# xiaoxiaokuye/CODLAD

Measured on NVIDIA B200. Metric: backmapped residues/sec (100-step, 10-ensemble), higher is better.
Workload: dtype f16 (tcgen05, fp32 accumulate)

## Files before the change

codlad_b200/csrc/capi.cu:

```cuda
#include <stdarg.h>
#include <string.h>

#include <map>
#include <string>
#include <vector>

#include "../../include/codlad_b200.h"
#include "decode.h"
#include "model.h"

namespace cb2 {

static thread_local char g_err[1024] = "";

void set_error(const char* fmt, ...) {
    va_list ap;
    va_start(ap, fmt);
    vsnprintf(g_err, sizeof(g_err), fmt, ap);
    va_end(ap);
}

float* plan_P(Plan& p, int which) { return p.P + (size_t)which * p.NB * p.L * 256; }

namespace {

struct TensorTable {
    std::map<std::string, const cb2_tensor*> by_name;
    TensorTable(const cb2_tensor* t, int n) {
        for (int i = 0; i < n; ++i) by_name[t[i].name] = &t[i];
    }
    const float* get(const std::string& name, long long numel) const {
        auto it = by_name.find(name);
        if (it == by_name.end()) { set_error("missing tensor '%s'", name.c_str()); return nullptr; }
        if (it->second->numel != numel) {
            set_error("tensor '%s': numel %lld, expected %lld", name.c_str(), it->second->numel, numel);
            return nullptr;
        }
        return it->second->data;
    }
};

struct Packer {
    std::vector<float> buf;
    size_t reserve(size_t n) {
        size_t off = (buf.size() + 63) & ~(size_t)63;
        buf.resize(off + n, 0.0f);
        return off;
    }
    size_t transposed(const float* W, int out, int in_total, int col0, int ncols, float scale = 1.0f) {
        size_t off = reserve((size_t)ncols * out);
        for (int k = 0; k < ncols; ++k)
            for (int o = 0; o < out; ++o) buf[off + (size_t)k * out + o] = scale * W[(size_t)o * in_total + col0 + k];
        return off;
    }
    size_t copy(const float* v, size_t n) {
        size_t off = reserve(n);
        memcpy(&buf[off], v, n * sizeof(float));
        return off;
    }
};

struct HalfPacker {
    std::vector<__half> buf;
    size_t block(const float* W, int in_total, int col0, float scale = 1.0f) {
        size_t off = buf.size();
        buf.resize(off + 128 * 128);
        for (int o = 0; o < 128; ++o)
            for (int k = 0; k < 128; ++k) buf[off + (size_t)o * 128 + k] = __float2half_rn(scale * W[(size_t)o * in_total + col0 + k]);
        return off;
    }
};

#define GET(var, name, numel)                               \
    const float* var = tt.get(name, (long long)(numel));    \
    if (!var) return 1;

template <typename T>
int dev_alloc(std::vector<void*>& owned, T** ptr, size_t count) {
    void* q = nullptr;
    CB2_CUDA(cudaMalloc(&q, count * sizeof(T) > 0 ? count * sizeof(T) : 16));
    owned.push_back(q);
    *ptr = reinterpret_cast<T*>(q);
    return 0;
}

}
}

using namespace cb2;

struct cb2_denoiser { DenoiserModel m; };
struct cb2_vae { VaeModel v; };
struct cb2_plan {
    Plan p;
    float* ca_full = nullptr;
    int *csr_row = nullptr, *csr_col = nullptr;
    int E = 0;
    signed char* orders = nullptr;
    int* slot_atom = nullptr;
    long long* out_off = nullptr;
    float *edge_w = nullptr, *S40 = nullptr, *phi = nullptr, *ic = nullptr, *zq = nullptr;
    int* vq_idx = nullptr;
    float *xa = nullptr, *xb = nullptr;
    int keep_debug = 0;
    bool frames_ready = false, topo_ready = false;
};

extern "C" {

int cb2_abi_version(void) { return CB2_ABI_VERSION; }
const char* cb2_last_error(void) { return cb2::g_err; }

int cb2_denoiser_create(const cb2_tensor* tensors, int n_tensors, const float* freqs128, int k_neighbors, cb2_denoiser** out) {
    if (!tensors || !freqs128 || !out) { set_error("denoiser_create: null argument"); return 1; }
    TensorTable tt(tensors, n_tensors);
    Packer pk;
    HalfPacker bp;
    const int H = CB2_H;
    std::map<std::string, size_t> off;
    std::map<std::string, size_t> boff;

    off["freqs"] = pk.copy(freqs128, 128);
    GET(te0w, "t_embedder.mlp.0.weight", H * 256) GET(te0b, "t_embedder.mlp.0.bias", H)
    GET(te2w, "t_embedder.mlp.2.weight", H * H) GET(te2b, "t_embedder.mlp.2.bias", H)
    off["te_w0_t"] = pk.transposed(te0w, H, 256, 0, 256); off["te_b0"] = pk.copy(te0b, H);
    off["te_w2_t"] = pk.transposed(te2w, H, H, 0, H); off["te_b2"] = pk.copy(te2b, H);

    {
        size_t wo = pk.reserve((size_t)H * CB2_MOD_TOTAL), bo = pk.reserve(CB2_MOD_TOTAL);
        off["ada_w_t"] = wo; off["ada_b"] = bo;
        int col = 0;
        auto put = [&](const std::string& pre, int width) -> int {
            const float* w = tt.get(pre + ".adaLN_modulation.1.weight", (long long)width * H);
            const float* b = tt.get(pre + ".adaLN_modulation.1.bias", width);
            if (!w || !b) return 1;
            for (int o = 0; o < width; ++o) {
                pk.buf[bo + col + o] = b[o];
                for (int k = 0; k < H; ++k) pk.buf[wo + (size_t)k * CB2_MOD_TOTAL + col + o] = w[(size_t)o * H + k];
            }
            col += width;
            return 0;
        };
        for (int l = 0; l < 3; ++l) if (put("encoder_layers." + std::to_string(l), CB2_MOD_ENC)) return 1;
        for (int l = 0; l < 3; ++l) if (put("decoder_layers." + std::to_string(l), CB2_MOD_DEC)) return 1;
        if (put("W_out", CB2_MOD_FIN)) return 1;
    }
    GET(xinw, "x_in.weight", H * 3) GET(xinb, "x_in.bias", H)
    off["xin_w_t"] = pk.transposed(xinw, H, 3, 0, 3); off["xin_b"] = pk.copy(xinb, H);

    GET(posw, "features.embeddings.linear.weight", 16 * 66) GET(posb, "features.embeddings.linear.bias", 16)
    GET(edgew, "features.edge_embedding.weight", H * 167)
    GET(lnw, "features.norm_edges.weight", H) GET(lnb, "features.norm_edges.bias", H)
    GET(wew, "W_e.weight", H * H) GET(web, "W_e.bias", H)
    {
        size_t o = pk.reserve(65 * H);
        for (int d = 0; d < 65; ++d)
            for (int c = 0; c < H; ++c) {
                double a = 0.0;
                for (int q = 0; q < 16; ++q) a += (double)(posw[q * 66 + d] + posb[q]) * (double)edgew[(size_t)c * 167 + q];
                pk.buf[o + (size_t)d * H + c] = (float)a;
            }
        off["pos_table"] = o;
        size_t w = pk.reserve(152 * H);
        for (int r = 0; r < 151; ++r)
            for (int c = 0; c < H; ++c) pk.buf[w + (size_t)r * H + c] = edgew[(size_t)c * 167 + 16 + r];
        off["wedge_t"] = w;
    }
    off["ln_w"] = pk.copy(lnw, H); off["ln_b"] = pk.copy(lnb, H);
    off["we_t"] = pk.transposed(wew, H, H, 0, H); off["we_b"] = pk.copy(web, H);

    GET(ws, "W_s.weight", 30 * H)
    for (int l = 0; l < 3; ++l) {
        const std::string p = "encoder_layers." + std::to_string(l), k = "e" + std::to_string(l) + ".";
        GET(w1, p + ".W1.weight", H * 3 * H) GET(b1, p + ".W1.bias", H) GET(w2, p + ".W2.weight", H * H) GET(b2, p + ".W2.bias", H)
        GET(w3, p + ".W3.weight", H * H) GET(b3, p + ".W3.bias", H)
        GET(w11, p + ".W11.weight", H * 3 * H) GET(b11, p + ".W11.bias", H) GET(w12, p + ".W12.weight", H * H) GET(b12, p + ".W12.bias", H)
        GET(w13, p + ".W13.weight", H * H) GET(b13, p + ".W13.bias", H)
        GET(win, p + ".dense.W_in.weight", 4 * H * H) GET(bin, p + ".dense.W_in.bias", 4 * H)
        GET(wout, p + ".dense.W_out.weight", H * 4 * H) GET(bout, p + ".dense.W_out.bias", H)
        off[k + "W1a_t"] = pk.transposed(w1, H, 3 * H, 0, H); off[k + "W1b_t"] = pk.transposed(w1, H, 3 * H, H, H);
        off[k + "W1c_t"] = pk.transposed(w1, H, 3 * H, 2 * H, H); off[k + "b1"] = pk.copy(b1, H);
        off[k + "W2_t"] = pk.transposed(w2, H, H, 0, H); off[k + "b2"] = pk.copy(b2, H);
        off[k + "W3_t"] = pk.transposed(w3, H, H, 0, H); off[k + "b3"] = pk.copy(b3, H);
        off[k + "W11a_t"] = pk.transposed(w11, H, 3 * H, 0, H); off[k + "W11b_t"] = pk.transposed(w11, H, 3 * H, H, H);
        off[k + "W11c_t"] = pk.transposed(w11, H, 3 * H, 2 * H, H); off[k + "b11"] = pk.copy(b11, H);
        off[k + "W12_t"] = pk.transposed(w12, H, H, 0, H); off[k + "b12"] = pk.copy(b12, H);
        off[k + "W13_t"] = pk.transposed(w13, H, H, 0, H); off[k + "b13"] = pk.copy(b13, H);
        off[k + "Win_t"] = pk.transposed(win, 4 * H, H, 0, H); off[k + "bin"] = pk.copy(bin, 4 * H);
        off[k + "Wout_t"] = pk.transposed(wout, H, 4 * H, 0, 4 * H); off[k + "bout"] = pk.copy(bout, H);
        boff[k + "W1b"] = bp.block(w1, 3 * H, H); boff[k + "W2"] = bp.block(w2, H, 0, 0.5f);
        boff[k + "W11b"] = bp.block(w11, 3 * H, H); boff[k + "W12"] = bp.block(w12, H, 0, 0.5f); boff[k + "W13"] = bp.block(w13, H, 0, 0.5f);
        boff[k + "W1a"] = bp.block(w1, 3 * H, 0); boff[k + "W1c"] = bp.block(w1, 3 * H, 2 * H);
        boff[k + "W11a"] = bp.block(w11, 3 * H, 0); boff[k + "W11c"] = bp.block(w11, 3 * H, 2 * H);
        boff[k + "W3"] = bp.block(w3, H, 0);
        for (int q = 0; q < 4; ++q) { size_t o = bp.block(win + (size_t)q * H * H, H, 0); if (q == 0) boff[k + "Win"] = o; }
        for (int q = 0; q < 4; ++q) { size_t o = bp.block(wout, 4 * H, q * H, 0.5f); if (q == 0) boff[k + "Wout"] = o; }
    }
    for (int l = 0; l < 3; ++l) {
        const std::string p = "decoder_layers." + std::to_string(l), k = "d" + std::to_string(l) + ".";
        GET(w1, p + ".W1.weight", H * 4 * H) GET(b1, p + ".W1.bias", H) GET(w2, p + ".W2.weight", H * H) GET(b2, p + ".W2.bias", H)
        GET(w3, p + ".W3.weight", H * H) GET(b3, p + ".W3.bias", H)
        GET(win, p + ".dense.W_in.weight", 4 * H * H) GET(bin, p + ".dense.W_in.bias", 4 * H)
        GET(wout, p + ".dense.W_out.weight", H * 4 * H) GET(bout, p + ".dense.W_out.bias", H)
        off[k + "W1a_t"] = pk.transposed(w1, H, 4 * H, 0, H); off[k + "W1b2_t"] = pk.transposed(w1, H, 4 * H, H, H, 2.0f);
        off[k + "W1d_t"] = pk.transposed(w1, H, 4 * H, 3 * H, H); off[k + "b1"] = pk.copy(b1, H);
        {
            size_t o = pk.reserve(30 * H);
            for (int z = 0; z < 30; ++z)
                for (int c = 0; c < H; ++c) {
                    double a = 0.0;
                    for (int q = 0; q < H; ++q) a += (double)ws[z * H + q] * (double)w1[(size_t)c * 4 * H + 2 * H + q];
                    pk.buf[o + (size_t)z * H + c] = (float)(2.0 * a);
                }
            off[k + "TS"] = o;
        }
        off[k + "W2_t"] = pk.transposed(w2, H, H, 0, H); off[k + "b2"] = pk.copy(b2, H);
        off[k + "W3_t"] = pk.transposed(w3, H, H, 0, H); off[k + "b3"] = pk.copy(b3, H);
        off[k + "Win_t"] = pk.transposed(win, 4 * H, H, 0, H); off[k + "bin"] = pk.copy(bin, 4 * H);
        off[k + "Wout_t"] = pk.transposed(wout, H, 4 * H, 0, 4 * H); off[k + "bout"] = pk.copy(bout, H);
        boff[k + "W1b2"] = bp.block(w1, 4 * H, H, 2.0f); boff[k + "W2"] = bp.block(w2, H, 0, 0.5f);
        boff[k + "W1a"] = bp.block(w1, 4 * H, 0); boff[k + "W1d"] = bp.block(w1, 4 * H, 3 * H);
        boff[k + "W3"] = bp.block(w3, H, 0);
        for (int q = 0; q < 4; ++q) { size_t o = bp.block(win + (size_t)q * H * H, H, 0); if (q == 0) boff[k + "Win"] = o; }
        for (int q = 0; q < 4; ++q) { size_t o = bp.block(wout, 4 * H, q * H, 0.5f); if (q == 0) boff[k + "Wout"] = o; }
    }
    GET(finw, "W_out.linear.weight", 6 * H) GET(finb, "W_out.linear.bias", 6)
    off["fin_w_t"] = pk.transposed(finw, 6, H, 0, H); off["fin_b"] = pk.copy(finb, 6);

    cb2_denoiser* d = new cb2_denoiser();
    DenoiserModel& m = d->m;
    m.k_neighbors = k_neighbors;
    CB2_CUDA(cudaMalloc(&m.dev_f32, pk.buf.size() * sizeof(float)));
    CB2_CUDA(cudaMemcpy(m.dev_f32, pk.buf.data(), pk.buf.size() * sizeof(float), cudaMemcpyHostToDevice));
    {
        std::vector<__half> v16;
        std::map<std::string, size_t> voff;
        auto putv = [&](const std::string& key, const float* src) {
            voff[key] = v16.size();
            for (int q = 0; q < H; ++q) v16.push_back(__float2half_rn(src[q]));
        };
        for (int l = 0; l < 3; ++l) {
            const std::string pe = "encoder_layers." + std::to_string(l), pd = "decoder_layers." + std::to_string(l);
            putv("e" + std::to_string(l) + ".b2", tt.get(pe + ".W2.bias", H));
            putv("e" + std::to_string(l) + ".b12", tt.get(pe + ".W12.bias", H));
            putv("e" + std::to_string(l) + ".b13", tt.get(pe + ".W13.bias", H));
            putv("d" + std::to_string(l) + ".b2", tt.get(pd + ".W2.bias", H));
        }
        CB2_CUDA(cudaMalloc(&m.dev_vec16, v16.size() * sizeof(__half)));
        CB2_CUDA(cudaMemcpy(m.dev_vec16, v16.data(), v16.size() * sizeof(__half), cudaMemcpyHostToDevice));
        for (int l = 0; l < 3; ++l) {
            m.enc[l].b2_16 = m.dev_vec16 + voff.at("e" + std::to_string(l) + ".b2");
            m.enc[l].b12_16 = m.dev_vec16 + voff.at("e" + std::to_string(l) + ".b12");
            m.enc[l].b13_16 = m.dev_vec16 + voff.at("e" + std::to_string(l) + ".b13");
            m.dec[l].b2_16 = m.dev_vec16 + voff.at("d" + std::to_string(l) + ".b2");
        }
    }
    CB2_CUDA(cudaMalloc(&m.dev_f16, bp.buf.size() * sizeof(__half)));
    CB2_CUDA(cudaMemcpy(m.dev_f16, bp.buf.data(), bp.buf.size() * sizeof(__half), cudaMemcpyHostToDevice));
    m.n_f16_blocks = (int)(bp.buf.size() / (128 * 128));
    auto F = [&](const std::string& key) { return (const float*)(m.dev_f32 + off.at(key)); };
    auto B = [&](const std::string& key) { return (const __half*)(m.dev_f16 + boff.at(key)); };
    m.freqs = F("freqs"); m.te_w0_t = F("te_w0_t"); m.te_b0 = F("te_b0"); m.te_w2_t = F("te_w2_t"); m.te_b2 = F("te_b2");
    m.ada_w_t = F("ada_w_t"); m.ada_b = F("ada_b"); m.xin_w_t = F("xin_w_t"); m.xin_b = F("xin_b");
    m.pos_table = F("pos_table"); m.wedge_t = F("wedge_t"); m.ln_w = F("ln_w"); m.ln_b = F("ln_b"); m.we_t = F("we_t"); m.we_b = F("we_b");
    for (int l = 0; l < 3; ++l) {
        const std::string k = "e" + std::to_string(l) + ".";
        EncLayerW& e = m.enc[l];
        e.W1a_t = F(k + "W1a_t"); e.W1b_t = F(k + "W1b_t"); e.W1c_t = F(k + "W1c_t"); e.b1 = F(k + "b1");
        e.W2_t = F(k + "W2_t"); e.b2 = F(k + "b2"); e.W3_t = F(k + "W3_t"); e.b3 = F(k + "b3");
        e.W11a_t = F(k + "W11a_t"); e.W11b_t = F(k + "W11b_t"); e.W11c_t = F(k + "W11c_t"); e.b11 = F(k + "b11");
        e.W12_t = F(k + "W12_t"); e.b12 = F(k + "b12"); e.W13_t = F(k + "W13_t"); e.b13 = F(k + "b13");
        e.Win_t = F(k + "Win_t"); e.bin = F(k + "bin"); e.Wout_t = F(k + "Wout_t"); e.bout = F(k + "bout");
        e.W1b_h = B(k + "W1b"); e.W2_h = B(k + "W2"); e.W11b_h = B(k + "W11b"); e.W12_h = B(k + "W12"); e.W13_h = B(k + "W13");
        e.W1a_h = B(k + "W1a"); e.W1c_h = B(k + "W1c"); e.W11a_h = B(k + "W11a"); e.W11c_h = B(k + "W11c");
        e.W3_h = B(k + "W3"); e.Win_h = B(k + "Win"); e.Wout_h = B(k + "Wout");
    }
    for (int l = 0; l < 3; ++l) {
        const std::string k = "d" + std::to_string(l) + ".";
        DecLayerW& e = m.dec[l];
        e.W1a_t = F(k + "W1a_t"); e.W1b2_t = F(k + "W1b2_t"); e.W1d_t = F(k + "W1d_t"); e.b1 = F(k + "b1"); e.TS = F(k + "TS");
        e.W2_t = F(k + "W2_t"); e.b2 = F(k + "b2"); e.W3_t = F(k + "W3_t"); e.b3 = F(k + "b3");
        e.Win_t = F(k + "Win_t"); e.bin = F(k + "bin"); e.Wout_t = F(k + "Wout_t"); e.bout = F(k + "bout");
        e.W1b2_h = B(k + "W1b2"); e.W2_h = B(k + "W2");
        e.W1a_h = B(k + "W1a"); e.W1d_h = B(k + "W1d"); e.W3_h = B(k + "W3"); e.Win_h = B(k + "Win"); e.Wout_h = B(k + "Wout");
    }
    m.fin_w_t = F("fin_w_t"); m.fin_b = F("fin_b");
    *out = d;
    return 0;
}

void cb2_denoiser_destroy(cb2_denoiser* d) {
    if (!d) return;
    cudaFree(d->m.dev_f32);
    cudaFree(d->m.dev_f16);
    cudaFree(d->m.dev_vec16);
    delete d;
}

int cb2_vae_create(const cb2_tensor* tensors, int n_tensors, const float* mean3, const float* std3, int angle_variant, cb2_vae** out) {
    if (!tensors || !mean3 || !std3 || !out) { set_error("vae_create: null argument"); return 1; }
    TensorTable tt(tensors, n_tensors);
    Packer pk;
    std::map<std::string, size_t> off;
    const std::string P = "equivaraintconv.";
    auto itcb = tt.by_name.find("quantize._codebook.embed");
    if (itcb == tt.by_name.end() || itcb->second->numel % 3 != 0) { set_error("missing/invalid quantize._codebook.embed"); return 1; }
    const int M = (int)(itcb->second->numel / 3);
    off["codebook"] = pk.copy(itcb->second->data, (size_t)M * 3);
    off["mean"] = pk.copy(mean3, 3); off["std"] = pk.copy(std3, 3);
    GET(mow, "map_out.weight", 36 * 3) GET(mob, "map_out.bias", 36)
    off["mapw_t"] = pk.transposed(mow, 36, 3, 0, 3); off["mapb"] = pk.copy(mob, 36);
    GET(remb, P + "res_embed.weight", 25 * 4) off["res_embed"] = pk.copy(remb, 100);
    const int D = 40, T = angle_variant ? 50 : 40;
    auto linear = [&](const std::string& key, const std::string& name, int o, int i) -> int {
        const float* w = tt.get(P + name + ".weight", (long long)o * i);
        const float* b = tt.get(P + name + ".bias", o);
        if (!w || !b) return 1;
        off[key + "_t"] = pk.transposed(w, o, i, 0, i);
        off[key + "_b"] = pk.copy(b, o);
        return 0;
    };
    size_t wd = pk.reserve(4 * 15 * D), bd = pk.reserve(4 * D);
    off["Wd_t"] = wd; off["bd"] = bd;
    for (int b = 0; b < 4; ++b) {
        const std::string s = std::to_string(b);
        if (linear("inv0." + s, "message_blocks." + s + ".inv_dense.0", D, D)) return 1;
        if (linear("inv1." + s, "message_blocks." + s + ".inv_dense.1", D, D)) return 1;
        GET(dw, P + "message_blocks." + s + ".dist_embed.block.1.weight", D * 15)
        GET(db, P + "message_blocks." + s + ".dist_embed.block.1.bias", D)
        for (int q = 0; q < 15; ++q)
            for (int c = 0; c < D; ++c) pk.buf[wd + ((size_t)b * 15 + q) * D + c] = dw[c * 15 + q];
        for (int c = 0; c < D; ++c) pk.buf[bd + b * D + c] = db[c];
        if (linear("db1." + s, "dense_blocks." + s + ".1", D, D)) return 1;
        if (linear("db3." + s, "dense_blocks." + s + ".3", D, D)) return 1;
        if (linear("tb1." + s, "sidechain_torsion_blocks." + s + ".1", T, T)) return 1;
        if (linear("tb3." + s, "sidechain_torsion_blocks." + s + ".3", T, T)) return 1;
    }
    GET(bbd, P + "backbone_dist.weight", 75) GET(scd, P + "sidechain_dist.weight", 250)
    off["bb_dist"] = pk.copy(bbd, 75); off["sc_dist"] = pk.copy(scd, 250);
    if (linear("ba1", "backbone_angle.1", 3, D) || linear("ba3", "backbone_angle.3", 3, 3)) return 1;
    if (linear("bt1", "backbone_torsion.1", 3, D + 3) || linear("bt3", "backbone_torsion.3", 3, 3)) return 1;
    if (angle_variant) {
        if (linear("sa1", "sidechain_angle.1", 10, D) || linear("sa3", "sidechain_angle.3", 10, 10)) return 1;
    } else {
        GET(sae, P + "sidechain_angle.weight", 250) off["sa_embed"] = pk.copy(sae, 250);
    }
    if (linear("ft1", "final_torsion.1", 10, T) || linear("ft3", "final_torsion.3", 10, 10)) return 1;

    cb2_vae* h = new cb2_vae();
    VaeModel& v = h->v;
    v.M = M; v.angle_variant = angle_variant;
    CB2_CUDA(cudaMalloc(&v.dev, pk.buf.size() * sizeof(float)));
    CB2_CUDA(cudaMemcpy(v.dev, pk.buf.data(), pk.buf.size() * sizeof(float), cudaMemcpyHostToDevice));
    auto F = [&](const std::string& key) -> const float* {
        auto it = off.find(key);
        return it == off.end() ? nullptr : (const float*)(v.dev + it->second);
    };
    v.codebook = F("codebook"); v.mean = F("mean"); v.stdv = F("std"); v.mapw_t = F("mapw_t"); v.mapb = F("mapb");
    v.res_embed = F("res_embed"); v.Wd_t = F("Wd_t"); v.bd = F("bd");
    for (int b = 0; b < 4; ++b) {
        const std::string s = std::to_string(b);
        v.inv0_t[b] = F("inv0." + s + "_t"); v.inv0_b[b] = F("inv0." + s + "_b");
        v.inv1_t[b] = F("inv1." + s + "_t"); v.inv1_b[b] = F("inv1." + s + "_b");
        v.db1_t[b] = F("db1." + s + "_t"); v.db1_b[b] = F("db1." + s + "_b");
        v.db3_t[b] = F("db3." + s + "_t"); v.db3_b[b] = F("db3." + s + "_b");
        v.tb1_t[b] = F("tb1." + s + "_t"); v.tb1_b[b] = F("tb1." + s + "_b");
        v.tb3_t[b] = F("tb3." + s + "_t"); v.tb3_b[b] = F("tb3." + s + "_b");
    }
    v.bb_dist = F("bb_dist"); v.sc_dist = F("sc_dist"); v.sa_embed = F("sa_embed");
    v.ba1_t = F("ba1_t"); v.ba1_b = F("ba1_b"); v.ba3_t = F("ba3_t"); v.ba3_b = F("ba3_b");
    v.bt1_t = F("bt1_t"); v.bt1_b = F("bt1_b"); v.bt3_t = F("bt3_t"); v.bt3_b = F("bt3_b");
    v.sa1_t = F("sa1_t"); v.sa1_b = F("sa1_b"); v.sa3_t = F("sa3_t"); v.sa3_b = F("sa3_b");
    v.ft1_t = F("ft1_t"); v.ft1_b = F("ft1_b"); v.ft3_t = F("ft3_t"); v.ft3_b = F("ft3_b");
    CB2_CUDA(cudaMalloc(&v.e2, (size_t)M * sizeof(float)));
    if (int e = launch_codebook_norms(v.codebook, M, v.e2, 0)) return e;
    CB2_CUDA(cudaStreamSynchronize(0));
    *out = h;
    return 0;
}

void cb2_vae_destroy(cb2_vae* h) {
    if (!h) return;
    cudaFree(h->v.dev);
    cudaFree(h->v.e2);
    delete h;
}

int cb2_plan_create(const cb2_denoiser* d, int F, int NB, int L, int precision, int keep_debug, cb2_plan** out) {
    if (!out || F <= 0 || NB <= 0 || L <= 0) { set_error("plan_create: bad argument"); return 1; }
    if (precision != PREC_F32 && precision != PREC_F16) { set_error("plan_create: unknown precision %d", precision); return 1; }
    cb2_plan* h = new cb2_plan();
    Plan& p = h->p;
    p.model = d ? &d->m : nullptr; p.F = F; p.NB = NB; p.L = L; p.precision = precision;
    h->keep_debug = keep_debug;
    if (!d) {
        int e = 0;
        e |= dev_alloc(p.allocs, &p.X, (size_t)F * L * 3);
        e |= dev_alloc(p.allocs, &p.lengths, F);
        e |= dev_alloc(p.allocs, &p.cg_z, (size_t)F * L);
        e |= dev_alloc(p.allocs, &p.frame_of, NB);
        if (e) { cb2_plan_destroy(h); return e; }
        *out = h;
        return 0;
    }
    p.K = d->m.k_neighbors < L ? d->m.k_neighbors : L;
    const size_t N = (size_t)NB * L, FE = (size_t)F * L * p.K, NE = N * p.K;
    const size_t esz = precision == PREC_F16 ? 2 : 4;
    int e = 0;
    e |= dev_alloc(p.allocs, &p.X, (size_t)F * L * 3);
    e |= dev_alloc(p.allocs, &p.lengths, F);
    e |= dev_alloc(p.allocs, &p.cg_z, (size_t)F * L);
    e |= dev_alloc(p.allocs, &p.frame_of, NB);
    e |= dev_alloc(p.allocs, &p.nbr_idx, FE);
    e |= dev_alloc(p.allocs, &p.nbr_dist, FE);
    e |= dev_alloc(p.allocs, reinterpret_cast<unsigned char**>(&p.hE0), FE * 128 * esz);
    e |= dev_alloc(p.allocs, reinterpret_cast<unsigned char**>(&p.hE), NE * 128 * esz);
    if (keep_debug) e |= dev_alloc(p.allocs, &p.E_dbg, FE * 128);
    e |= dev_alloc(p.allocs, &p.hV, N * 128);
    e |= dev_alloc(p.allocs, &p.hVenc, N * 128);
    e |= dev_alloc(p.allocs, &p.P, 2 * N * 256);
    if (precision == PREC_F16) {
        e |= dev_alloc(p.allocs, &p.P16[0], N * 256);
        e |= dev_alloc(p.allocs, &p.P16[1], N * 256);
    }
    e |= dev_alloc(p.allocs, &p.S, N * 128);
    e |= dev_alloc(p.allocs, &p.out6, N * 6);
    e |= dev_alloc(p.allocs, &h->xa, N * 3);
    e |= dev_alloc(p.allocs, &h->xb, N * 3);
    p.mod_capacity = NB > 1024 ? NB : 1024;
    e |= dev_alloc(p.allocs, &p.mod, (size_t)p.mod_capacity * CB2_MOD_TOTAL);
    if (precision == PREC_F16) e |= dev_alloc(p.allocs, &p.mod16, (size_t)p.mod_capacity * 768);
    e |= dev_alloc(p.allocs, &p.silu_c, (size_t)p.mod_capacity * 128);
    e |= dev_alloc(p.allocs, &p.tvals, p.mod_capacity);
    e |= dev_alloc(p.allocs, &p.coef, (size_t)p.mod_capacity * 8);
    if (e) { cb2_plan_destroy(h); return e; }
    if (precision == PREC_F16) {
        if (int r = edge_tc_prepare(p)) { cb2_plan_destroy(h); return r; }
        if (int r = node_tc_prepare(p)) { cb2_plan_destroy(h); return r; }
    }
    *out = h;
    return 0;
}

void cb2_plan_destroy(cb2_plan* h) {
    if (!h) return;
    if (h->p.graph) cudaGraphExecDestroy(h->p.graph);
    edge_tc_release(h->p);
    node_tc_release(h->p);
    for (void* q : h->p.allocs) cudaFree(q);
    delete h;
}

int cb2_plan_K(const cb2_plan* h) { return h ? h->p.K : 0; }
long long cb2_plan_launches(const cb2_plan* h) { return h ? h->p.launches : 0; }

int cb2_plan_set_frames(cb2_plan* h, const float* X, const int* lengths, const int* cg_z, const int* frame_of, void* stream) {
    if (!h || !X || !lengths || !cg_z || !frame_of) { set_error("set_frames: null argument"); return 1; }
    Plan& p = h->p;
    cudaStream_t s = (cudaStream_t)stream;
    CB2_CUDA(cudaMemcpyAsync(p.X, X, (size_t)p.F * p.L * 3 * sizeof(float), cudaMemcpyDeviceToDevice, s));
    CB2_CUDA(cudaMemcpyAsync(p.lengths, lengths, p.F * sizeof(int), cudaMemcpyDeviceToDevice, s));
    CB2_CUDA(cudaMemcpyAsync(p.cg_z, cg_z, (size_t)p.F * p.L * sizeof(int), cudaMemcpyDeviceToDevice, s));
    CB2_CUDA(cudaMemcpyAsync(p.frame_of, frame_of, p.NB * sizeof(int), cudaMemcpyDeviceToDevice, s));
    if (p.model == nullptr) { h->frames_ready = true; return 0; }
    {
        std::vector<int> len((size_t)p.F);
        CB2_CUDA(cudaMemcpyAsync(len.data(), p.lengths, (size_t)p.F * sizeof(int), cudaMemcpyDeviceToHost, s));
        CB2_CUDA(cudaStreamSynchronize(s));
        p.all_full = true;
        for (int f = 0; f < p.F; ++f) p.all_full = p.all_full && len[f] >= p.L;
    }
    if (int e = launch_knn(p.X, p.lengths, p.F, p.L, p.K, p.nbr_dist, p.nbr_idx, s)) return e;
    if (int e = launch_edge_features(*p.model, p.X, p.lengths, p.nbr_idx, p.nbr_dist, p.F, p.L, p.K, p.E_dbg, p.hE0, p.precision, s)) return e;
    p.launches += 2;
    h->frames_ready = true;
    return 0;
}

}

namespace {

int edge_dispatch(Plan& p, int mode, int layer, const float* mod_base, int mod_stride, cudaStream_t s) {
    return p.precision == PREC_F16 ? launch_edge_tc(p, mode, layer, mod_base, mod_stride, s)
                                    : launch_edge_f32(p, mode, layer, mod_base, mod_stride, s);
}

int run_forward(Plan& p, const float* x, const float* mod_base, int mod_stride, const float* noise, float* x_next,
                const float* coef_row, cudaStream_t s, int stop_after = -1) {
    int n = 0;
    auto done = [&]() { return stop_after >= 0 && ++n >= stop_after; };
    const bool tc = p.precision == PREC_F16 && p.node_tc != nullptr;
    auto node_update = [&](int phase, const float* xt, const float* nz, float* xn, const float* cf) {
        return tc ? launch_node_update_tc(p, phase, mod_base, mod_stride, xt, nz, xn, cf, s)
                  : launch_node_update(p, phase, mod_base, mod_stride, xt, nz, xn, cf, s);
    };
    if (int e = tc ? launch_node_init_tc(p, x, s) : launch_node_init(p, x, mod_base, mod_stride, s)) return e;
    if (done()) return 0;
    for (int l = 0; l < 3; ++l) {
        if (int e = edge_dispatch(p, EDGE_ENC_NODE, l, mod_base, mod_stride, s)) return e;
        if (done()) return 0;
        if (int e = node_update(l, nullptr, nullptr, nullptr, nullptr)) return e;
        if (done()) return 0;
        if (int e = edge_dispatch(p, EDGE_ENC_EDGE, l, mod_base, mod_stride, s)) return e;
        if (done()) return 0;
    }
    for (int l = 0; l < 3; ++l) {
        if (int e = edge_dispatch(p, EDGE_DEC, l, mod_base, mod_stride, s)) return e;
        if (done()) return 0;
        const bool last = l == 2;
        if (int e = node_update(3 + l, last ? x : nullptr, last ? noise : nullptr, last ? x_next : nullptr, last ? coef_row : nullptr)) return e;
        if (done()) return 0;
    }
    return 0;
}

}

extern "C" {

int cb2_plan_forward_partial(cb2_plan* h, const float* x, const float* t, int stop_after, void* stream) {
    if (!h || !x || !t) { set_error("forward_partial: null argument"); return 1; }
    if (!h->frames_ready || !h->p.model) { set_error("forward_partial: no denoiser frames on this plan"); return 1; }
    Plan& p = h->p;
    cudaStream_t s = (cudaStream_t)stream;
    if (int e = launch_timestep_mod(*p.model, t, p.NB, p.silu_c, p.mod, p.mod16, s)) return e;
    p.coef_steps = 0;
    return run_forward(p, x, p.mod, CB2_MOD_TOTAL, nullptr, nullptr, nullptr, s, stop_after);
}

int cb2_plan_forward(cb2_plan* h, const float* x, const float* t, float* out, void* stream) {
    if (!h || !x || !t || !out) { set_error("forward: null argument"); return 1; }
    if (!h->frames_ready || !h->p.model) { set_error("forward: cb2_plan_set_frames has not been called (or decode-only plan)"); return 1; }
    Plan& p = h->p;
    cudaStream_t s = (cudaStream_t)stream;
    if (p.NB > p.mod_capacity) { set_error("forward: NB exceeds table capacity"); return 1; }
    if (int e = launch_timestep_mod(*p.model, t, p.NB, p.silu_c, p.mod, p.mod16, s)) return e;
    p.launches += 2;
    p.coef_steps = 0;
    if (int e = run_forward(p, x, p.mod, CB2_MOD_TOTAL, nullptr, nullptr, nullptr, s)) return e;
    CB2_CUDA(cudaMemcpyAsync(out, p.out6, (size_t)p.NB * p.L * 6 * sizeof(float), cudaMemcpyDeviceToDevice, s));
    return 0;
}

static int set_schedule(cb2_plan* h, const float* t_of_step, const float* coef, int T, int kind, cudaStream_t s) {
    if (!h || !t_of_step || !coef || T <= 0 || !h->p.model) { set_error("set_schedule: bad argument"); return 1; }
    Plan& p = h->p;
    if (T > p.mod_capacity) { set_error("set_schedule: T=%d exceeds capacity %d", T, p.mod_capacity); return 1; }
    CB2_CUDA(cudaMemcpyAsync(p.tvals, t_of_step, T * sizeof(float), cudaMemcpyHostToDevice, s));
    CB2_CUDA(cudaMemcpyAsync(p.coef, coef, (size_t)T * 8 * sizeof(float), cudaMemcpyHostToDevice, s));
    if (int e = launch_timestep_mod(*p.model, p.tvals, T, p.silu_c, p.mod, p.mod16, s)) return e;
    CB2_CUDA(cudaStreamSynchronize(s));
    p.launches += 2;
    p.coef_steps = T;
    p.update_kind = kind;
    p.coef_noisy = kind == UPDATE_DDPM;
    for (int i = 0; i < T && !p.coef_noisy; ++i) p.coef_noisy = coef[(size_t)i * 8 + 4] != 0.0f;
    if (p.graph) { cudaGraphExecDestroy(p.graph); p.graph = nullptr; }
    return 0;
}

int cb2_plan_set_schedule(cb2_plan* h, const float* t_of_step, const float* coef, int T, void* stream) {
    return set_schedule(h, t_of_step, coef, T, UPDATE_DDPM, (cudaStream_t)stream);
}

int cb2_plan_set_ddim_schedule(cb2_plan* h, const float* t_of_step, const float* ddim_coef, int T, void* stream) {
    return set_schedule(h, t_of_step, ddim_coef, T, UPDATE_DDIM, (cudaStream_t)stream);
}

static int enqueue_loop(cb2_plan* h, float* x, const float* noise, cudaStream_t s) {
    Plan& p = h->p;
    const size_t n3 = (size_t)p.NB * p.L * 3;
    CB2_CUDA(cudaMemcpyAsync(h->xa, x, n3 * sizeof(float), cudaMemcpyDeviceToDevice, s));
    float *cur = h->xa, *nxt = h->xb;
    for (int step = p.coef_steps - 1; step >= 0; --step) {
        const float* mod_row = p.mod + (size_t)step * CB2_MOD_TOTAL;
        const float* step_noise = noise != nullptr ? noise + (size_t)step * n3 : nullptr;
        if (int e = run_forward(p, cur, mod_row, 0, step_noise, nxt, p.coef + (size_t)step * 8, s)) {
            char prev[1024];
            snprintf(prev, sizeof(prev), "%s", g_err);
            const unsigned int* tl = edge_tc_trap_log();
            if (tl != nullptr) {
                char w[600]; int n = 0;
                for (int i = 0; i < 18 && n < 560; ++i)
                    if (tl[4 + 2 * i]) n += snprintf(w + n, sizeof(w) - n, " w%d:bar+0x%x/p%u", i, tl[4 + 2 * i] & 0xfffu, tl[5 + 2 * i] >> 16);
                set_error("%s [sampling step %d; block %u timed-out waits:%s]", prev, step, tl[0] - 1u, w);
            }
            else set_error("%s [sampling step %d]", prev, step);
            return e;
        }
        float* t = cur; cur = nxt; nxt = t;
    }
    CB2_CUDA(cudaMemcpyAsync(x, cur, n3 * sizeof(float), cudaMemcpyDeviceToDevice, s));
    return 0;
}

int cb2_plan_sample(cb2_plan* h, float* x, const float* noise, int use_graph, void* stream) {
    if (!h || !x) { set_error("sample: null argument"); return 1; }
    Plan& p = h->p;
    if (!h->frames_ready || p.coef_steps <= 0) { set_error("sample: set_frames / set_schedule must be called first"); return 1; }
    if (!noise && p.coef_noisy) { set_error("sample: noise may be NULL only on a DDIM schedule whose sigma are all zero (eta = 0)"); return 1; }
    cudaStream_t s = (cudaStream_t)stream;
    if (!use_graph) return enqueue_loop(h, x, noise, s);
    if (!p.graph || p.graph_key[0] != x || p.graph_key[1] != noise || p.graph_steps != p.coef_steps || p.graph_all_full != p.all_full) {
        if (p.graph) { cudaGraphExecDestroy(p.graph); p.graph = nullptr; }
        cudaStream_t cs;
        CB2_CUDA(cudaStreamCreateWithFlags(&cs, cudaStreamNonBlocking));
        const long long before = p.launches;
        CB2_CUDA(cudaStreamBeginCapture(cs, cudaStreamCaptureModeThreadLocal));
        int e = enqueue_loop(h, x, noise, cs);
        cudaGraph_t g = nullptr;
        cudaError_t ce = cudaStreamEndCapture(cs, &g);
        p.launches = before;
        if (e || ce != cudaSuccess) {
            if (g) cudaGraphDestroy(g);
            cudaStreamDestroy(cs);
            if (!e) set_error("graph capture failed: %s", cudaGetErrorString(ce));
            return e ? e : (int)ce;
        }
        ce = cudaGraphInstantiate(&p.graph, g, 0);
        cudaGraphDestroy(g);
        cudaStreamDestroy(cs);
        if (ce != cudaSuccess) { set_error("graph instantiate failed: %s", cudaGetErrorString(ce)); p.graph = nullptr; return (int)ce; }
        p.graph_key[0] = x; p.graph_key[1] = noise; p.graph_steps = p.coef_steps; p.graph_all_full = p.all_full;
    }
    CB2_CUDA(cudaGraphLaunch(p.graph, s));
    p.launches += 16LL * p.coef_steps;
    return 0;
}

int cb2_plan_set_topology(cb2_plan* h, const cb2_vae* v, const float* ca_full, const int* csr_row_ptr, const int* csr_col,
                          int n_edges, const signed char* atom_orders, const int* slot_atom, const long long* out_offset,
                          void* stream) {
    if (!h || !v || !ca_full || !csr_row_ptr || !atom_orders || !slot_atom || !out_offset) { set_error("set_topology: null argument"); return 1; }
    Plan& p = h->p;
    cudaStream_t s = (cudaStream_t)stream;
    const size_t N = (size_t)p.NB * p.L, FL = (size_t)p.F * p.L;
    if (!h->ca_full) {
        int e = 0;
        e |= dev_alloc(p.allocs, &h->ca_full, (size_t)p.F * (p.L + 2) * 3);
        e |= dev_alloc(p.allocs, &h->csr_row, FL + 1);
        e |= dev_alloc(p.allocs, &h->orders, FL * 30);
        e |= dev_alloc(p.allocs, &h->slot_atom, FL * 14);
        e |= dev_alloc(p.allocs, &h->out_off, p.NB);
        e |= dev_alloc(p.allocs, &h->S40, N * 40);
        e |= dev_alloc(p.allocs, &h->phi, N * 40);
        e |= dev_alloc(p.allocs, &h->ic, N * 39);
        e |= dev_alloc(p.allocs, &h->zq, N * 3);
        e |= dev_alloc(p.allocs, &h->vq_idx, N);
        if (e) return e;
    }
    if (n_edges > h->E || !h->csr_col) {
        int e = dev_alloc(p.allocs, &h->csr_col, (size_t)n_edges);
        e |= dev_alloc(p.allocs, &h->edge_w, (size_t)4 * n_edges * 40);
        if (e) return e;
    }
    h->E = n_edges;
    CB2_CUDA(cudaMemcpyAsync(h->ca_full, ca_full, (size_t)p.F * (p.L + 2) * 3 * sizeof(float), cudaMemcpyDeviceToDevice, s));
    CB2_CUDA(cudaMemcpyAsync(h->csr_row, csr_row_ptr, (FL + 1) * sizeof(int), cudaMemcpyDefault, s));
    if (n_edges) CB2_CUDA(cudaMemcpyAsync(h->csr_col, csr_col, (size_t)n_edges * sizeof(int), cudaMemcpyDefault, s));
    CB2_CUDA(cudaMemcpyAsync(h->orders, atom_orders, FL * 30, cudaMemcpyDefault, s));
    CB2_CUDA(cudaMemcpyAsync(h->slot_atom, slot_atom, FL * 14 * sizeof(int), cudaMemcpyDefault, s));
    CB2_CUDA(cudaMemcpyAsync(h->out_off, out_offset, p.NB * sizeof(long long), cudaMemcpyDefault, s));
    if (!h->frames_ready) { set_error("set_topology: call cb2_plan_set_frames first (needs X)"); return 1; }
    if (int e = launch_ic_edge_filters(v->v, p.X, p.F, p.L, h->csr_row, h->csr_col, n_edges, h->edge_w, s)) return e;
    p.launches += 1;
    CB2_CUDA(cudaStreamSynchronize(s));
    h->topo_ready = true;
    return 0;
}

int cb2_plan_decode(cb2_plan* h, const cb2_vae* v, const float* latent, int denorm, int* idx, float* zq, float* ic_recon,
                    float* xyz, void* stream) {
    if (!h || !v || !latent) { set_error("decode: null argument"); return 1; }
    if (!h->topo_ready) { set_error("decode: cb2_plan_set_topology has not been called"); return 1; }
    Plan& p = h->p;
    cudaStream_t s = (cudaStream_t)stream;
    const int N = p.NB * p.L;
    if (int e = launch_vq_lookup(v->v, latent, N, p.L, p.lengths, p.frame_of, denorm, h->vq_idx, h->zq, h->S40, s)) return e;
    if (int e = launch_ic_decoder(v->v, h->S40, h->phi, N, p.L, p.frame_of, p.lengths, p.cg_z, h->csr_row, h->csr_col, h->E,
                                  h->edge_w, h->ic, s, &p.launches)) return e;
    p.launches += 1;
    if (idx) CB2_CUDA(cudaMemcpyAsync(idx, h->vq_idx, (size_t)N * sizeof(int), cudaMemcpyDeviceToDevice, s));
    if (zq) CB2_CUDA(cudaMemcpyAsync(zq, h->zq, (size_t)N * 3 * sizeof(float), cudaMemcpyDeviceToDevice, s));
    if (ic_recon) CB2_CUDA(cudaMemcpyAsync(ic_recon, h->ic, (size_t)N * 39 * sizeof(float), cudaMemcpyDeviceToDevice, s));
    if (xyz) {
        if (int e = launch_ic_to_xyz(h->ca_full, h->ic, N, p.L, p.frame_of, p.lengths, h->orders, h->slot_atom, h->out_off, xyz,
                                     nullptr, s)) return e;
        p.launches += 1;
    }
    return 0;
}

int cb2_plan_buffer(cb2_plan* h, const char* name, void* dst, long long dst_bytes, void* stream) {
    if (!h || !name || !dst) { set_error("plan_buffer: null argument"); return 1; }
    void* src = nullptr;
    long long size = 0;
    void** ptr = &src;
    long long* bytes = &size;
    Plan& p = h->p;
    const size_t N = (size_t)p.NB * p.L, FE = (size_t)p.F * p.L * p.K, esz = p.precision == PREC_F16 ? 2 : 4;
    const std::string n = name;
    if (n == "nbr_idx") { *ptr = p.nbr_idx; *bytes = FE * 4; }
    else if (n == "nbr_dist") { *ptr = p.nbr_dist; *bytes = FE * 4; }
    else if (n == "E") { *ptr = p.E_dbg; *bytes = p.E_dbg ? FE * 128 * 4 : 0; }
    else if (n == "hE0") { *ptr = p.hE0; *bytes = FE * 128 * esz; }
    else if (n == "hE") { *ptr = p.hE; *bytes = N * p.K * 128 * esz; }
    else if (n == "hV") { *ptr = p.hV; *bytes = N * 128 * 4; }
    else if (n == "S") { *ptr = p.S; *bytes = N * 128 * 4; }
    else if (n == "out6") { *ptr = p.out6; *bytes = N * 6 * 4; }
    else if (n == "tc_trace") {
        if (!p.tc_trace) { unsigned long long* t = nullptr; if (dev_alloc(p.allocs, &t, 6144)) return 1; cudaMemsetAsync(t, 0, 49152, (cudaStream_t)stream); p.tc_trace = t; }
        *ptr = p.tc_trace; *bytes = 49152;
    }
    else if (n == "mod") { *ptr = p.mod; *bytes = (size_t)p.mod_capacity * CB2_MOD_TOTAL * 4; }
    else { set_error("plan_buffer: unknown buffer '%s'", name); return 1; }
    if (!src || dst_bytes > size) { set_error("plan_buffer: '%s' holds %lld bytes, %lld requested", name, size, dst_bytes); return 1; }
    CB2_CUDA(cudaMemcpyAsync(dst, src, (size_t)dst_bytes, cudaMemcpyDeviceToDevice, (cudaStream_t)stream));
    return 0;
}

int cb2_plan_run_edge_kernel(cb2_plan* h, int mode, int layer, void* stream) {
    if (!h || mode < 0 || mode > 2 || layer < 0 || layer > 2) { set_error("run_edge_kernel: bad argument"); return 1; }
    if (!h->frames_ready || h->p.coef_steps <= 0) { set_error("run_edge_kernel: set_frames / set_schedule first"); return 1; }
    return edge_dispatch(h->p, mode, layer, h->p.mod, 0, (cudaStream_t)stream);
}

int cb2_plan_run_stage(cb2_plan* h, const cb2_vae* v, int stage, int layer, float* xyz_scratch, void* stream) {
    if (!h || stage < 0 || stage > 9) { set_error("run_stage: bad argument"); return 1; }
    Plan& p = h->p;
    cudaStream_t s = (cudaStream_t)stream;
    if (!h->frames_ready) { set_error("run_stage: set_frames first"); return 1; }
    if (stage <= 3 && (p.coef_steps <= 0 || !p.model)) { set_error("run_stage: set_schedule first"); return 1; }
    if (stage >= 6 && (!h->topo_ready || !v)) { set_error("run_stage: set_topology first (and pass the vae)"); return 1; }
    const int N = p.NB * p.L;
    switch (stage) {
        case 0: case 1: case 2:
            if (layer < 0 || layer > 2) { set_error("run_stage: layer"); return 1; }
            return edge_dispatch(p, stage, layer, p.mod, 0, s);
        case 3: {
            if (layer < 0 || layer > 5) { set_error("run_stage: phase"); return 1; }
            const bool last = layer == 5, tc = p.precision == PREC_F16 && p.node_tc != nullptr;
            const float *xt = last ? h->xa : nullptr, *nz = last ? h->xa : nullptr, *cf = last ? p.coef : nullptr;
            float* xn = last ? h->xb : nullptr;
            return tc ? launch_node_update_tc(p, layer, p.mod, 0, xt, nz, xn, cf, s) : launch_node_update(p, layer, p.mod, 0, xt, nz, xn, cf, s);
        }
        case 4: return launch_knn(p.X, p.lengths, p.F, p.L, p.K, p.nbr_dist, p.nbr_idx, s);
        case 5: return launch_edge_features(*p.model, p.X, p.lengths, p.nbr_idx, p.nbr_dist, p.F, p.L, p.K, p.E_dbg, p.hE0, p.precision, s);
        case 6: return launch_vq_lookup(v->v, h->xa, N, p.L, p.lengths, p.frame_of, 1, h->vq_idx, h->zq, h->S40, s);
        case 7: return launch_ic_decoder(v->v, h->S40, h->phi, N, p.L, p.frame_of, p.lengths, p.cg_z, h->csr_row, h->csr_col, h->E, h->edge_w, h->ic, s, &p.launches);
        case 8:
            if (!xyz_scratch) { set_error("run_stage: ic_to_xyz needs xyz_scratch"); return 1; }
            return launch_ic_to_xyz(h->ca_full, h->ic, N, p.L, p.frame_of, p.lengths, h->orders, h->slot_atom, h->out_off, xyz_scratch, nullptr, s);
        default: return launch_ic_edge_filters(v->v, p.X, p.F, p.L, h->csr_row, h->csr_col, h->E, h->edge_w, s);
    }
}

int cb2_knn_topk(const float* X, const int* lengths, int F, int L, int K, float* D, int* idx, void* stream) {
    if (!X || !D || !idx) { set_error("knn_topk: null argument"); return 1; }
    return launch_knn(X, lengths, F, L, K, D, idx, (cudaStream_t)stream);
}

int cb2_vq_lookup(const cb2_vae* v, const float* x, int NB, int L, const int* lengths, const int* frame_of, int denorm,
                  int* idx, float* zq, void* stream) {
    if (!v || !x || !lengths || !frame_of || !idx || !zq) { set_error("vq_lookup: null argument"); return 1; }
    return launch_vq_lookup(v->v, x, NB * L, L, lengths, frame_of, denorm, idx, zq, nullptr, (cudaStream_t)stream);
}

int cb2_p_sample(const float* x, const float* model_out, const float* noise, const float* coef, const int* step_of_member,
                 int rows_per_member, int rows, int C, float* x_next, void* stream) {
    if (!x || !model_out || !noise || !coef || !step_of_member || !x_next) { set_error("p_sample: null argument"); return 1; }
    return launch_p_sample(x, model_out, noise, coef, step_of_member, rows_per_member, rows, C, x_next, (cudaStream_t)stream);
}

int cb2_ddim_sample(const float* x, const float* model_out, const float* noise, const float* coef, const int* step_of_member,
                    int rows_per_member, int rows, int C, float* x_next, void* stream) {
    if (!x || !model_out || !coef || !step_of_member || !x_next) { set_error("ddim_sample: null argument"); return 1; }
    return launch_ddim_sample(x, model_out, noise, coef, step_of_member, rows_per_member, rows, C, x_next, (cudaStream_t)stream);
}

int cb2_ic_to_xyz(const float* ca_full, const float* ic_recon, int NB, int L, const int* frame_of, const int* lengths,
                  const signed char* atom_orders, const int* slot_atom, const long long* out_offset, float* xyz, void* stream) {
    if (!ca_full || !ic_recon || !frame_of || !lengths || !atom_orders || !slot_atom || !out_offset || !xyz) {
        set_error("ic_to_xyz: null argument");
        return 1;
    }
    return launch_ic_to_xyz(ca_full, ic_recon, NB * L, L, frame_of, lengths, atom_orders, slot_atom, out_offset, xyz, nullptr,
                            (cudaStream_t)stream);
}

}
```

codlad_b200/csrc/edge_tc.cu:

```cuda
#include <cstring>
#include "model.h"
#include "tc_common.cuh"

namespace cb2 {

using namespace tc;

namespace {

constexpr int IND_BYTES = 16 * 128 * 2;
constexpr int MAX_NPT = 4;

struct TcMaps {
    CUtensorMap in_frame;
    CUtensorMap state;
    CUtensorMap weights;
};

struct TcParams {
    int L, K, NPT, tiles_per_member, n_tiles;
    int in_is_frame;
    int single_frame;
    int w_row[3];
    int n_w;
    const __half* P16;
    const __half* b2h;
    const __half* b3h;
    const __half* mod16;
    int mod16_stride;
    const __half* res;
    __half* out;
    const int *lengths, *frame_of, *nbr_idx;
    float* S;
    unsigned long long* trace;
    int trace_slot;
    int trace_epi;
};

#ifndef CB2_EPI_SUBS
#define CB2_EPI_SUBS 1
#endif
constexpr int SUBS = CB2_EPI_SUBS;
constexpr int NCG = 4 / SUBS;
constexpr int EPI_THREADS = 128 * NCG;
constexpr int CTA_THREADS = EPI_THREADS + 64;
constexpr int NSLOT = 4;

__device__ __forceinline__ void row_quarter_sync(int q) { asm volatile("bar.sync %0, %1;" ::"r"(q + 1), "n"(32 * NCG) : "memory"); }

struct TileMeta { uint32_t a, b; };
__device__ __forceinline__ int meta_member(const TileMeta& m) { return (int)(m.a >> 16); }
__device__ __forceinline__ int meta_tin(const TileMeta& m) { return (int)(m.a & 0xffffu); }
__device__ __forceinline__ int meta_j(const TileMeta& m) { return (int)(m.b & 0x7fffffffu); }
__device__ __forceinline__ bool meta_row_valid(const TileMeta& m) { return (int)m.b >= 0; }

template <int MODE, bool MASKED>
__global__ void __launch_bounds__(CTA_THREADS, 1) edge_tc_kernel(const __grid_constant__ TcMaps maps, const TcParams p) {
    extern __shared__ __align__(1024) unsigned char smem[];
    constexpr int N_W = MODE == EDGE_ENC_EDGE ? 3 : 2;
    unsigned char* sW = smem;
    unsigned char* sT = sW + N_W * TILE_BYTES;
    unsigned char* sAux = sT + 4 * TILE_BYTES;
    unsigned char* sInd = sAux;
    uint64_t* sBar = reinterpret_cast<uint64_t*>(sAux + (MODE == EDGE_ENC_EDGE ? 0 : IND_BYTES));
    uint32_t* sTmem = reinterpret_cast<uint32_t*>(sBar + 29);

    const int tid = threadIdx.x;
    if (tid == 0) trace_window(p.trace, p.trace_slot, false);
    const int K = p.K, NPT = p.NPT;
    if ((smem_u32(smem) & 1023u) != 0) __trap();
    pdl_launch_dependents();

    if (tid == 0) {
        mbar_init(smem_u32(&sBar[0]), 1);
        for (int g = 0; g < 4; ++g) {
            mbar_init(smem_u32(&sBar[1 + 3 * g]), 1);
            mbar_init(smem_u32(&sBar[2 + 3 * g]), 1);
            mbar_init(smem_u32(&sBar[3 + 3 * g]), EPI_THREADS / 32);
            mbar_init(smem_u32(&sBar[13 + g]), 1);
            mbar_init(smem_u32(&sBar[17 + g]), 1);
            mbar_init(smem_u32(&sBar[21 + g]), 1);
            mbar_init(smem_u32(&sBar[25 + g]), 4);
        }
        asm volatile("fence.mbarrier_init.release.cluster;" ::: "memory");
    }
    if (tid >= EPI_THREADS && tid < EPI_THREADS + 32) {
        asm volatile("tcgen05.alloc.cta_group::1.sync.aligned.shared::cta.b32 [%0], 512;" ::"r"(smem_u32(sTmem)) : "memory");
        asm volatile("tcgen05.relinquish_alloc_permit.cta_group::1.sync.aligned;" ::: "memory");
    }
    if (MODE != EDGE_ENC_EDGE) {
        for (int t = tid; t < 16 * 16; t += CTA_THREADS) {
            const int q = t >> 4, c16 = t & 15;
            uint32_t w[4];
#pragma unroll
            for (int e = 0; e < 4; ++e) {
                const int r0 = c16 * 8 + e * 2;
                const __half lo = __float2half((q < NPT && r0 / K == q) ? 0.5f : 0.f);
                const __half hi = __float2half((q < NPT && (r0 + 1) / K == q) ? 0.5f : 0.f);
                w[e] = (uint32_t)__half_as_ushort(lo) | ((uint32_t)__half_as_ushort(hi) << 16);
            }
            const uint32_t off = (uint32_t)((c16 >> 3) * (16 * 128) + q * 128 + (((c16 & 7) ^ (q & 7)) << 4));
            *reinterpret_cast<uint4*>(sInd + off) = make_uint4(w[0], w[1], w[2], w[3]);
        }
    }
    fence_async_smem();
    tc_fence_before();
    __syncthreads();
    tc_fence_after();
    const uint32_t tmem_base = *sTmem;
    const int tile_begin = (int)((long long)blockIdx.x * p.n_tiles / gridDim.x);
    const int tile_end = (int)((long long)(blockIdx.x + 1) * p.n_tiles / gridDim.x);
    constexpr int tile_stride = 4;
    constexpr uint32_t IDESC_MAIN = umma_idesc(128, 128, 0, 0);
    constexpr uint32_t IDESC_RED = umma_idesc(128, 16, 1, 0);

    if (tid >= EPI_THREADS) {
        auto T_u32 = [&](int g) { return smem_u32(sT + g * TILE_BYTES); };
#ifdef CB2_TRACE_CTRL
        unsigned long long* ctr = (p.trace != nullptr && blockIdx.x == 0 && (tid & 31) == 0) ? p.trace + (tid >= EPI_THREADS + 32 ? 5632 : 5120) : nullptr;
        int n_ctr = 0;
        auto cmark = [&](int ev, int g) {
            if (ctr != nullptr && n_ctr < 500) {
                unsigned long long t;
                asm volatile("mov.u64 %0, %%globaltimer;" : "=l"(t));
                ctr[1 + n_ctr] = (t << 8) | (unsigned long long)((ev << 2) | g);
                ctr[0] = (unsigned long long)(++n_ctr);
            }
        };
#else
        auto cmark = [](int, int) {};
#endif
        auto bar_load = [&](int g) { return smem_u32(&sBar[1 + 3 * g]); };
        auto bar_acc = [&](int g) { return smem_u32(&sBar[2 + 3 * g]); };
        auto bar_epi = [&](int g) { return smem_u32(&sBar[3 + 3 * g]); };
        auto bar_go = [&](int g) { return smem_u32(&sBar[13 + g]); };
        auto bar_m3 = [&](int g) { return smem_u32(&sBar[17 + g]); };
        auto bar_res = [&](int g) { return smem_u32(&sBar[21 + g]); };
        if (tid >= EPI_THREADS + 32) {
            const CUtensorMap* in_map = p.in_is_frame ? &maps.in_frame : &maps.state;
            if (elect_one()) {
                mbar_expect_tx(smem_u32(&sBar[0]), (uint32_t)(N_W * TILE_BYTES));
                for (int m = 0; m < N_W; ++m)
                    for (int h = 0; h < 2; ++h)
                        tma_load_2d(smem_u32(sW + m * TILE_BYTES + h * HALF_BYTES), &maps.weights, h * 64, p.w_row[m], smem_u32(&sBar[0]));
            }
            __syncwarp();
            int nv[4], out_row0[4], in_row0[4];
            auto issue_rows = [&](int g, uint32_t bar) {
                if (elect_one()) {
                    mbar_expect_tx(bar, (uint32_t)(nv[g] * K * 256));
                    for (int q = 0; q < nv[g]; ++q)
                        for (int h = 0; h < 2; ++h)
                            tma_load_2d(T_u32(g) + h * HALF_BYTES + q * K * 128, in_map, h * 64, in_row0[g] + q * K, bar);
                }
                __syncwarp();
            };
            auto issue_load = [&](int g, int t) {
                const int b = t / p.tiles_per_member;
                const int i0 = (t - b * p.tiles_per_member) * NPT;
                nv[g] = min(NPT, p.L - i0);
                in_row0[g] = ((p.in_is_frame ? __ldg(p.frame_of + b) : b) * p.L + i0) * K;
                out_row0[g] = (b * p.L + i0) * K;
                issue_rows(g, bar_load(g));
            };
            pdl_wait();
            for (int g = 0; g < 4; ++g)
                if (tile_begin + g < tile_end) issue_load(g, tile_begin + g);
            uint32_t ph_go = 0;
            for (int t0 = tile_begin; t0 < tile_end; t0 += tile_stride) {
                if (MODE == EDGE_ENC_EDGE) {
                    for (int g = 0; g < 4 && t0 + g < tile_end; ++g) { mbar_wait(bar_m3(g), ph_go); issue_rows(g, bar_res(g)); }
                }
                for (int g = 0; g < 4; ++g) {
                    const int t = t0 + g;
                    if (t >= tile_end) break;
                    mbar_wait(bar_go(g), ph_go);
                    cmark(0, g);
                    if (MODE == EDGE_ENC_EDGE) {
                        if (elect_one()) {
                            for (int q = 0; q < nv[g]; ++q)
                                for (int h = 0; h < 2; ++h)
                                    tma_store_2d(&maps.state, h * 64, out_row0[g] + q * K, T_u32(g) + h * HALF_BYTES + q * K * 128);
                            tma_store_commit();
                        }
                        __syncwarp();
                    }
                    if (t + tile_stride < tile_end) {
                        if (MODE == EDGE_ENC_EDGE) { if (elect_one()) tma_store_wait_read(); __syncwarp(); }
                        issue_load(g, t + tile_stride);
                        cmark(1, g);
                    }
                }
                ph_go ^= 1;
            }
            if (MODE == EDGE_ENC_EDGE) { if (elect_one()) tma_store_wait_all(); __syncwarp(); }
        } else {
            uint32_t ph_epi = 0;
            auto issue_mma = [&](int g, int w_slot) {
                tc_fence_after();
                const uint64_t a0 = umma_desc(T_u32(g), 16, 1024), b0 = umma_desc(smem_u32(sW + w_slot * TILE_BYTES), 16, 1024);
                if (elect_one()) {
#pragma unroll
                    for (int k = 0; k < 8; ++k) {
                        const uint64_t koff = (uint64_t)(((k >> 2) * HALF_BYTES + (k & 3) * 32) >> 4);
                        umma_f16(tmem_base + (uint32_t)(g * 128), a0 + koff, b0 + koff, IDESC_MAIN, k > 0);
                    }
                    umma_commit(bar_acc(g));
                }
                __syncwarp();
            };
            auto issue_reduce = [&](int g) {
                tc_fence_after();
                const uint64_t a0 = umma_desc(T_u32(g), HALF_BYTES, 1024), b0 = umma_desc(smem_u32(sInd), 16, 1024);
                if (elect_one()) {
#pragma unroll
                    for (int k = 0; k < 8; ++k)
                        umma_f16(tmem_base + (uint32_t)(g * 128), a0 + (uint64_t)((k * 16 * 128) >> 4),
                                 b0 + (uint64_t)(((k >> 2) * (16 * 128) + (k & 3) * 32) >> 4), IDESC_RED, k > 0);
                    umma_commit(bar_acc(g));
                    umma_commit(bar_go(g));
                }
                __syncwarp();
            };
            cmark(6, 0);
            mbar_wait(smem_u32(&sBar[0]), 0);
            cmark(7, 0);
            uint32_t round = 0;
            if (MODE == EDGE_ENC_EDGE) {
                for (int t0 = tile_begin; t0 < tile_end; t0 += tile_stride, ++round) {
                    const int n = min(4, tile_end - t0);
                    const int n_next = max(0, min(4, tile_end - (t0 + tile_stride)));
                    if (round == 0)
                        for (int g = 0; g < n; ++g) { mbar_wait(bar_load(g), 0); issue_mma(g, 0); }
                    for (int g = 0; g < n; ++g) { mbar_wait(bar_epi(g), ph_epi); cmark(0, g); issue_mma(g, 1); cmark(1, g); }
                    ph_epi ^= 1;
                    for (int g = 0; g < n; ++g) {
                        mbar_wait(bar_epi(g), ph_epi);
                        cmark(2, g);
                        issue_mma(g, 2);
                        if (elect_one()) umma_commit(bar_m3(g));
                        __syncwarp();
                    }
                    ph_epi ^= 1;
                    const uint32_t next_parity = (round + 1) & 1;
                    for (int g = 0; g < n; ++g) {
                        mbar_wait(bar_epi(g), ph_epi);
                        if (elect_one()) mbar_arrive(bar_go(g));
                        __syncwarp();
                        cmark(3, g);
                        if (g >= 1 && g - 1 < n_next) { mbar_wait(bar_load(g - 1), next_parity); cmark(4, g - 1); issue_mma(g - 1, 0); cmark(5, g - 1); }
                    }
                    if (n - 1 < n_next) { mbar_wait(bar_load(n - 1), next_parity); issue_mma(n - 1, 0); }
                    ph_epi ^= 1;
                }
            } else {
                bool pend3 = false;
                uint32_t pend_round = 0;
                auto restart = [&](int h, uint32_t rnd) {
                    mbar_wait(smem_u32(&sBar[25 + h]), rnd & 1);
                    cmark(3, h);
                    mbar_wait(bar_load(h), (rnd + 1) & 1);
                    cmark(4, h);
                    issue_mma(h, 0);
                    cmark(5, h);
                };
                for (int t0 = tile_begin; t0 < tile_end; t0 += tile_stride, ++round) {
                    const int n = min(4, tile_end - t0);
                    const int n_next = max(0, min(4, tile_end - (t0 + tile_stride)));
                    if (round == 0)
                        for (int g = 0; g < n; ++g) { mbar_wait(bar_load(g), 0); issue_mma(g, 0); }
                    for (int g = 0; g < n; ++g) {
                        mbar_wait(bar_epi(g), ph_epi); cmark(0, g); issue_mma(g, 1); cmark(1, g);
                        if (g == 0 && pend3) { restart(3, pend_round); pend3 = false; }
                    }
                    ph_epi ^= 1;
                    for (int g = 0; g < n; ++g) {
                        mbar_wait(bar_epi(g), ph_epi);
                        cmark(2, g);
                        issue_reduce(g);
                        if (g >= 1 && g - 1 < n_next) restart(g - 1, round);
                    }
                    ph_epi ^= 1;
                    if (n - 1 < n_next) {
                        if (n == 4) { pend3 = true; pend_round = round; }
                        else restart(n - 1, round);
                    }
                }
            }
        }
    } else {
        const int warp = tid >> 5, quarter = warp & 3, cq = warp >> 2, r = quarter * 32 + (tid & 31);
        const int c0 = cq * 32 * SUBS;
        const int q_of_r = r / K;
        const int len0 = __ldg(p.lengths);
        const uint32_t tmem_lane = tmem_base + ((uint32_t)(quarter * 32) << 16) + (uint32_t)c0;
        auto stage_done = [&](int s, bool wrote_smem) {
            if (wrote_smem) fence_async_smem();
            tc_fence_before();
            __syncwarp();
            if ((tid & 31) == 0) mbar_arrive(smem_u32(&sBar[3 + 3 * s]));
        };

        const int step_b = tile_stride / p.tiles_per_member, step_t = tile_stride - step_b * p.tiles_per_member;
        auto make_meta = [&](int tile, int b, int tin) {
            TileMeta m{((uint32_t)b << 16) | (uint32_t)tin, 0x80000000u};
            if (tile >= tile_end) { m.a = 0u; return m; }
            const int i0 = tin * NPT;
            const int f = p.single_frame ? 0 : __ldg(p.frame_of + b);
            if (q_of_r < min(NPT, p.L - i0))
                m.b = (uint32_t)__ldg(p.nbr_idx + ((size_t)f * p.L + i0 + q_of_r) * K + (r - q_of_r * K));
            return m;
        };
        auto first_meta = [&](int tile) {
            const int b = tile / p.tiles_per_member;
            return make_meta(tile, b, tile - b * p.tiles_per_member);
        };
        auto next_meta = [&](const TileMeta& m, int tile) {
            int b = meta_member(m) + step_b, tin = meta_tin(m) + step_t;
            if (tin >= p.tiles_per_member) { tin -= p.tiles_per_member; ++b; }
            return make_meta(tile, b, tin);
        };
        auto node0_of = [&](const TileMeta& m) { return meta_member(m) * p.L + meta_tin(m) * NPT; };
        auto nv_of = [&](const TileMeta& m) { return min(NPT, p.L - meta_tin(m) * NPT); };
        auto row_keep = [&](const TileMeta& m) -> uint32_t {
            if (!meta_row_valid(m)) return 0u;
            if (MODE == EDGE_DEC) return 0xffffffffu;
            const int len = p.single_frame ? len0 : __ldg(p.lengths + __ldg(p.frame_of + meta_member(m)));
            return (meta_tin(m) * NPT + q_of_r < len && meta_j(m) < len) ? 0xffffffffu : 0u;
        };
        auto ld_pc = [&](const TileMeta& m, int col, uint32_t (&pc)[16]) {
#ifdef CB2_X_NOGATHER
            const __half* src = p.P16 + 128 + col;
#else
            const __half* src = p.P16 + ((size_t)meta_member(m) * p.L + meta_j(m)) * 256 + 128 + col;
#endif
            ldg256(src, *reinterpret_cast<uint32_t(*)[8]>(&pc[0]));
            ldg256(src + 16, *reinterpret_cast<uint32_t(*)[8]>(&pc[8]));
        };
        auto st16 = [&](unsigned char* T, int col, int g16, const uint32_t (&o)[8]) {
            *reinterpret_cast<uint4*>(T + tile_off(r, (col >> 3) + g16 * 2)) = make_uint4(o[0], o[1], o[2], o[3]);
            *reinterpret_cast<uint4*>(T + tile_off(r, (col >> 3) + g16 * 2 + 1)) = make_uint4(o[4], o[5], o[6], o[7]);
        };

#ifdef CB2_TRACE_EPI
        unsigned long long* trace = (p.trace != nullptr && p.trace_epi && blockIdx.x == 0 && tid == 0) ? p.trace : nullptr;
        int n_trace = 0;
        auto mark = [&](int ev, int s) {
            if (trace != nullptr && n_trace < 500) {
                unsigned long long t;
                asm volatile("mov.u64 %0, %%globaltimer;" : "=l"(t));
                trace[1 + n_trace] = (t << 8) | (unsigned long long)((ev << 2) | s);
                trace[0] = (unsigned long long)(++n_trace);
            }
        };
#else
        auto mark = [](int, int) {};
#endif
        TileMeta m0 = first_meta(tile_begin + 0), m1 = first_meta(tile_begin + 1), m2 = first_meta(tile_begin + 2), m3 = first_meta(tile_begin + 3);
        auto rotate = [&]() { const TileMeta t = m0; m0 = m1; m1 = m2; m2 = m3; m3 = t; };
        uint32_t ph = 0;
        uint32_t ph_res = 0;
        pdl_wait();

        auto drain = [&](int s, int next_tile) {
            const TileMeta m = m3;
            m3 = next_meta(m, next_tile);
            if (cq == s % NCG) {
                mark(8, s);
                mbar_wait(smem_u32(&sBar[2 + 3 * s]), ph ^ 1);
                tc_fence_after();
                mark(9, s);
                float s4[4];
                tmem_ld4(tmem_lane - (uint32_t)c0 + (uint32_t)(s * 128), s4);
                const int nv = nv_of(m), node0 = node0_of(m);
#pragma unroll
                for (int q = 0; q < MAX_NPT; ++q)
                    if (q < nv) p.S[((size_t)node0 + q) * 128 + r] = s4[q];
                tc_fence_before();
                __syncwarp();
                if ((tid & 31) == 0) mbar_arrive(smem_u32(&sBar[25 + s]));
                mark(10, s);
            }
        };
        bool pending3 = false;

        for (int t0 = tile_begin; t0 < tile_end; t0 += tile_stride) {
            const int n = min(NSLOT, tile_end - t0);
            auto epi1 = [&](int s) {
                unsigned char* T = sT + s * TILE_BYTES;
                uint32_t pc[SUBS][16];
                uint32_t pa[SUBS][16];
                const __half* pa_src = p.P16 + (size_t)(node0_of(m0) + (meta_row_valid(m0) ? q_of_r : 0)) * 256 + c0;
#pragma unroll
                for (int sub = 0; sub < SUBS; ++sub) {
                    ld_pc(m0, c0 + sub * 32, pc[sub]);
                    ldg256(pa_src + sub * 32, *reinterpret_cast<uint32_t(*)[8]>(&pa[sub][0]));
                    ldg256(pa_src + sub * 32 + 16, *reinterpret_cast<uint32_t(*)[8]>(&pa[sub][8]));
                }
                mark(0, s);
                if (MODE != EDGE_ENC_EDGE && cq != s % NCG && t0 != tile_begin) mbar_wait(smem_u32(&sBar[25 + s]), ph ^ 1);
                mbar_wait(smem_u32(&sBar[2 + 3 * s]), ph);
                tc_fence_after();
                mark(1, s);
#pragma unroll
                for (int sub = 0; sub < SUBS; ++sub) {
                    float acc0[16], acc1[16];
#ifdef CB2_X_NOLDTM
#pragma unroll
                    for (int e = 0; e < 16; ++e) {
                        asm volatile("mov.b32 %0, %1;" : "=f"(acc0[e]) : "r"(tid + e));
                        asm volatile("mov.b32 %0, %1;" : "=f"(acc1[e]) : "r"(tid - e));
                    }
#else
                    tmem_ld16x2(tmem_lane + (uint32_t)(s * 128 + sub * 32), acc0, acc1);
#endif
#pragma unroll
                    for (int g16 = 0; g16 < 2; ++g16) {
                        const float (&acc)[16] = g16 ? acc1 : acc0;
                        uint32_t o[8];
#pragma unroll
                        for (int e = 0; e < 8; ++e) {
                            const __half2 x = __hadd2(__hadd2(as_h2(pack_sat(acc[e * 2], acc[e * 2 + 1])), as_h2(pa[sub][g16 * 8 + e])), as_h2(pc[sub][g16 * 8 + e]));
                            o[e] = as_u32(gelu2_h2(x));
                        }
#ifdef CB2_X_NOSTS
                        if (o[0] == 0x12345678u && o[5] == 0x9abcdef0u) st16(T, c0 + sub * 32, g16, o);
#else
                        st16(T, c0 + sub * 32, g16, o);
#endif
                    }
                }
                mark(2, s);
                stage_done(s, true);
                mark(3, s);
            };
#pragma unroll 1
            for (int s = 0; s < NSLOT; ++s) {
                if (s < n) epi1(s);
                if (MODE != EDGE_ENC_EDGE && s == 0 && pending3) { drain(3, t0 + 3); pending3 = false; }
                rotate();
            }
            ph ^= 1;
#pragma unroll 1
            for (int s = 0; s < NSLOT; ++s) {
                if (s < n) {
                    unsigned char* T = sT + s * TILE_BYTES;
                    constexpr bool masked = MODE != EDGE_ENC_EDGE && MASKED;
                    const uint32_t keep = masked ? row_keep(m0) : 0xffffffffu;
                    uint32_t bb[SUBS][16];
#pragma unroll
                    for (int sub = 0; sub < SUBS; ++sub) {
                        ldg256(p.b2h + c0 + sub * 32, *reinterpret_cast<uint32_t(*)[8]>(&bb[sub][0]));
                        ldg256(p.b2h + c0 + sub * 32 + 16, *reinterpret_cast<uint32_t(*)[8]>(&bb[sub][8]));
                    }
                    mark(4, s);
                    mbar_wait(smem_u32(&sBar[2 + 3 * s]), ph);
                    tc_fence_after();
                    mark(5, s);
#pragma unroll
                    for (int sub = 0; sub < SUBS; ++sub) {
                        float acc0[16], acc1[16];
#ifdef CB2_X_NOLDTM
#pragma unroll
                        for (int e = 0; e < 16; ++e) {
                            asm volatile("mov.b32 %0, %1;" : "=f"(acc0[e]) : "r"(tid + e));
                            asm volatile("mov.b32 %0, %1;" : "=f"(acc1[e]) : "r"(tid - e));
                        }
#else
                        tmem_ld16x2(tmem_lane + (uint32_t)(s * 128 + sub * 32), acc0, acc1);
#endif
#pragma unroll
                        for (int g16 = 0; g16 < 2; ++g16) {
                            const float (&acc)[16] = g16 ? acc1 : acc0;
                            uint32_t o[8];
#pragma unroll
                            for (int e = 0; e < 8; ++e) {
                                const __half2 x = __hadd2(as_h2(pack_sat(acc[e * 2], acc[e * 2 + 1])), as_h2(bb[sub][g16 * 8 + e]));
                                o[e] = as_u32(gelu2_h2(x));
                            }
                            if (masked) {
#pragma unroll
                                for (int e = 0; e < 8; ++e) o[e] &= keep;
                            }
#ifdef CB2_X_NOSTS
                            if (o[0] == 0x12345678u && o[5] == 0x9abcdef0u) st16(T, c0 + sub * 32, g16, o);
#else
                            st16(T, c0 + sub * 32, g16, o);
#endif
                        }
                    }
                    mark(6, s);
                    stage_done(s, true);
                    mark(7, s);
                }
                if (MODE != EDGE_ENC_EDGE && s >= 1 && s - 1 < n) drain(s - 1, t0 + tile_stride + s - 1);
                rotate();
            }
            if (MODE != EDGE_ENC_EDGE) pending3 = n == NSLOT;
            ph ^= 1;
#pragma unroll 1
            for (int s = 0; s < NSLOT; ++s) {
                if (MODE == EDGE_ENC_EDGE && s < n) {
                    const TileMeta m = m0;
                    mark(8, s);
                    m0 = next_meta(m, t0 + tile_stride + s);
                    {
                        unsigned char* T = sT + s * TILE_BYTES;
                        const int bmem = meta_member(m);
                        mbar_wait(smem_u32(&sBar[2 + 3 * s]), ph);
                        tc_fence_after();
                        mbar_wait(smem_u32(&sBar[21 + s]), ph_res);
                        float sum = 0.f, sq = 0.f;
                        uint32_t v16[SUBS][16];
#pragma unroll
                        for (int sub = 0; sub < SUBS; ++sub) {
                            const int col = c0 + sub * 32;
                            uint32_t rs[16];
#pragma unroll
                            for (int c16 = 0; c16 < 4; ++c16) {
                                const uint4 t4 = *reinterpret_cast<const uint4*>(T + tile_off(r, (col >> 3) + c16));
                                rs[c16 * 4] = t4.x; rs[c16 * 4 + 1] = t4.y; rs[c16 * 4 + 2] = t4.z; rs[c16 * 4 + 3] = t4.w;
                            }
                            uint32_t b3r[16];
                            ldg256(p.b3h + col, *reinterpret_cast<uint32_t(*)[8]>(&b3r[0]));
                            ldg256(p.b3h + col + 16, *reinterpret_cast<uint32_t(*)[8]>(&b3r[8]));
#pragma unroll
                            for (int g16 = 0; g16 < 2; ++g16) {
                                float acc[16];
                                tmem_ld16(tmem_lane + (uint32_t)(s * 128 + sub * 32 + g16 * 16), acc);
#pragma unroll
                                for (int e = 0; e < 8; ++e) {
                                    const __half2 v = __hadd2(as_h2(rs[g16 * 8 + e]), __hadd2(as_h2(pack_sat(acc[e * 2], acc[e * 2 + 1])), as_h2(b3r[g16 * 8 + e])));
                                    const float2 vf = __half22float2(v);
                                    sum += vf.x + vf.y;
                                    sq = fmaf(vf.x, vf.x, fmaf(vf.y, vf.y, sq));
                                    v16[sub][g16 * 8 + e] = as_u32(v);
                                }
                            }
                        }
#ifdef CB2_X_NOXCHG
                        const float tsum = 4.0f * sum, tsq = 4.0f * sq;
#else
                        tmem_st2(tmem_lane + (uint32_t)(s * 128), sum, sq);
                        tc_fence_before();
                        row_quarter_sync(quarter);
                        tc_fence_after();
                        float part[8];
                        if (SUBS == 1) {
                            tmem_ld2_x4(tmem_base + ((uint32_t)(quarter * 32) << 16) + (uint32_t)(s * 128), 32u, part);
                        } else {
                            uint32_t r4[4];
                            const uint32_t ta = tmem_base + ((uint32_t)(quarter * 32) << 16) + (uint32_t)(s * 128);
                            asm volatile("tcgen05.ld.sync.aligned.32x32b.x2.b32 {%0,%1}, [%2];" : "=r"(r4[0]), "=r"(r4[1]) : "r"(ta));
                            asm volatile("tcgen05.ld.sync.aligned.32x32b.x2.b32 {%0,%1}, [%2];" : "=r"(r4[2]), "=r"(r4[3]) : "r"(ta + 64u));
                            asm volatile("tcgen05.wait::ld.sync.aligned;" ::: "memory");
#pragma unroll
                            for (int i = 0; i < 4; ++i) part[i] = __uint_as_float(r4[i]);
                            part[4] = part[5] = part[6] = part[7] = 0.f;
                        }
                        const float tsum = (part[0] + part[2]) + (part[4] + part[6]), tsq = (part[1] + part[3]) + (part[5] + part[7]);
#endif
                        const float mean = tsum * (1.0f / 128.0f);
                        const float rstd = rsqrtf(fmaxf(tsq * (1.0f / 128.0f) - mean * mean, 0.f) + 1e-6f);
                        const __half2 rstd2 = __float2half2_rn(rstd), nmr2 = __float2half2_rn(-mean * rstd);
#pragma unroll
                        for (int sub = 0; sub < SUBS; ++sub) {
                            const int col = c0 + sub * 32;
                            const __half* mod_row = p.mod16 + (size_t)bmem * p.mod16_stride + col;
#pragma unroll
                            for (int c16 = 0; c16 < 4; ++c16) {
                                const uint4 av = __ldg(reinterpret_cast<const uint4*>(mod_row + c16 * 8));
                                const uint4 bv = __ldg(reinterpret_cast<const uint4*>(mod_row + 128 + c16 * 8));
                                const uint32_t a4[4] = {av.x, av.y, av.z, av.w}, b4[4] = {bv.x, bv.y, bv.z, bv.w};
                                uint32_t o[4];
#pragma unroll
                                for (int e = 0; e < 4; ++e)
                                    o[e] = as_u32(__hfma2(__hfma2(as_h2(v16[sub][c16 * 4 + e]), rstd2, nmr2), as_h2(a4[e]), as_h2(b4[e])));
                                *reinterpret_cast<uint4*>(T + tile_off(r, (col >> 3) + c16)) = make_uint4(o[0], o[1], o[2], o[3]);
                            }
                        }
                        stage_done(s, true);
                        mark(9, s);
                    }
                }
                if (MODE == EDGE_ENC_EDGE) rotate();
            }
            ph ^= 1;
            ph_res ^= 1;
        }
        if (MODE != EDGE_ENC_EDGE && pending3) drain(3, tile_end);
    }
    tc_fence_before();
    __syncthreads();
    if (tid == 0) trace_window(p.trace, p.trace_slot, true);
    if (tid >= EPI_THREADS && tid < EPI_THREADS + 32) asm volatile("tcgen05.dealloc.cta_group::1.sync.aligned.b32 %0, 512;" ::"r"(tmem_base) : "memory");
}

}
}
namespace cb2 {
namespace {
#ifdef CB2_WITH_WG
#include "edge_wg.cuh"
#endif

size_t tc_smem_bytes(int mode) {
    const int n_w = mode == EDGE_ENC_EDGE ? 3 : 2;
    return (size_t)(n_w + 4) * TILE_BYTES + (mode == EDGE_ENC_EDGE ? 0 : IND_BYTES) + 29 * 8 + 16;
}

}

unsigned int* g_trap_host = nullptr;

const unsigned int* edge_tc_trap_log() { return g_trap_host; }

int edge_tc_prepare(Plan& p) {
    if (p.K > 128 || p.K < 1) { set_error("edge_tc: K=%d unsupported", p.K); return 1; }
    EncodeTiledFn fn = nullptr;
    if (get_encode_fn(&fn)) return 1;
    TcMaps* m = new TcMaps();
    p.tmaps = m;
    if (encode_rows_map(fn, &m->in_frame, p.hE0, (size_t)p.F * p.L * p.K, p.K)) return 1;
    if (encode_rows_map(fn, &m->state, p.hE, (size_t)p.NB * p.L * p.K, p.K)) return 1;
    if (encode_rows_map(fn, &m->weights, p.model->dev_f16, (size_t)p.model->n_f16_blocks * 128, 128)) return 1;
    if (getenv("CB2_TRAP_DEBUG") != nullptr && g_trap_host == nullptr) {
        unsigned int* dptr = nullptr;
        CB2_CUDA(cudaHostAlloc(&g_trap_host, 256, cudaHostAllocMapped));
        memset(g_trap_host, 0, 256);
        CB2_CUDA(cudaHostGetDevicePointer(&dptr, g_trap_host, 0));
        CB2_CUDA(cudaMemcpyToSymbol(tc::g_trap_log, &dptr, sizeof(dptr)));
    }
    int dev = 0;
    CB2_CUDA(cudaGetDevice(&dev));
    CB2_CUDA(cudaDeviceGetAttribute(&p.num_sms, cudaDevAttrMultiProcessorCount, dev));
    CB2_CUDA(cudaFuncSetAttribute(edge_tc_kernel<EDGE_ENC_NODE, false>, cudaFuncAttributeMaxDynamicSharedMemorySize, (int)tc_smem_bytes(EDGE_ENC_NODE)));
    CB2_CUDA(cudaFuncSetAttribute(edge_tc_kernel<EDGE_ENC_NODE, true>, cudaFuncAttributeMaxDynamicSharedMemorySize, (int)tc_smem_bytes(EDGE_ENC_NODE)));
    CB2_CUDA(cudaFuncSetAttribute(edge_tc_kernel<EDGE_DEC, false>, cudaFuncAttributeMaxDynamicSharedMemorySize, (int)tc_smem_bytes(EDGE_DEC)));
    CB2_CUDA(cudaFuncSetAttribute(edge_tc_kernel<EDGE_DEC, true>, cudaFuncAttributeMaxDynamicSharedMemorySize, (int)tc_smem_bytes(EDGE_DEC)));
    CB2_CUDA(cudaFuncSetAttribute(edge_tc_kernel<EDGE_ENC_EDGE, false>, cudaFuncAttributeMaxDynamicSharedMemorySize, (int)tc_smem_bytes(EDGE_ENC_EDGE)));
#ifdef CB2_WITH_WG
    CB2_CUDA(cudaFuncSetAttribute(wg::edge_wg_kernel<EDGE_ENC_NODE, false>, cudaFuncAttributeMaxDynamicSharedMemorySize, (int)wg::wg_smem_bytes(EDGE_ENC_NODE)));
    CB2_CUDA(cudaFuncSetAttribute(wg::edge_wg_kernel<EDGE_ENC_NODE, true>, cudaFuncAttributeMaxDynamicSharedMemorySize, (int)wg::wg_smem_bytes(EDGE_ENC_NODE)));
    CB2_CUDA(cudaFuncSetAttribute(wg::edge_wg_kernel<EDGE_DEC, false>, cudaFuncAttributeMaxDynamicSharedMemorySize, (int)wg::wg_smem_bytes(EDGE_DEC)));
    CB2_CUDA(cudaFuncSetAttribute(wg::edge_wg_kernel<EDGE_DEC, true>, cudaFuncAttributeMaxDynamicSharedMemorySize, (int)wg::wg_smem_bytes(EDGE_DEC)));
    CB2_CUDA(cudaFuncSetAttribute(wg::edge_wg_kernel<EDGE_ENC_EDGE, false>, cudaFuncAttributeMaxDynamicSharedMemorySize, (int)wg::wg_smem_bytes(EDGE_ENC_EDGE)));
#endif
    return 0;
}

void edge_tc_release(Plan& p) {
    delete reinterpret_cast<TcMaps*>(p.tmaps);
    p.tmaps = nullptr;
}

int launch_edge_tc(Plan& p, int mode, int layer, const float* mod_base, int mod_stride_b, cudaStream_t s) {
    const DenoiserModel& m = *p.model;
    const TcMaps& maps = *reinterpret_cast<const TcMaps*>(p.tmaps);
    TcParams tp{};
    tp.L = p.L; tp.K = p.K;
    if (p.NB > 65535 || p.L > 65535) { set_error("edge_tc: NB=%d / L=%d exceed the 16-bit tile metadata fields", p.NB, p.L); return 1; }
    tp.NPT = 128 / p.K < MAX_NPT ? 128 / p.K : MAX_NPT;
    if (tp.NPT < 1 || p.K % 8 != 0) tp.NPT = 1;
    tp.tiles_per_member = (p.L + tp.NPT - 1) / tp.NPT;
    tp.n_tiles = tp.tiles_per_member * p.NB;
    tp.lengths = p.lengths; tp.frame_of = p.frame_of; tp.nbr_idx = p.nbr_idx; tp.S = p.S;
    tp.trace = p.tc_trace; tp.trace_slot = p.launches & 2047;
    { static const bool ctrl_only = getenv("CB2_TRACE_CTRL_ONLY") != nullptr; tp.trace_epi = ctrl_only ? 0 : 1; }
    const bool first = (layer == 0 && mode != EDGE_DEC);
    tp.in_is_frame = first ? 1 : 0;
    tp.single_frame = p.F == 1 ? 1 : 0;
    const bool masked = tp.NPT * p.K < 128 || p.L % tp.NPT != 0 || (mode != EDGE_DEC && !p.all_full);
    auto row_of = [&](const __half* w) { return (int)((w - m.dev_f16) / 128); };
    if (mode == EDGE_ENC_NODE) {
        const EncLayerW& e = m.enc[layer];
        tp.P16 = p.P16[0]; tp.n_w = 2;
        tp.w_row[0] = row_of(e.W1b_h); tp.w_row[1] = row_of(e.W2_h); tp.b2h = e.b2_16;
    } else if (mode == EDGE_ENC_EDGE) {
        const EncLayerW& e = m.enc[layer];
        tp.P16 = p.P16[1]; tp.n_w = 3;
        tp.w_row[0] = row_of(e.W11b_h); tp.w_row[1] = row_of(e.W12_h); tp.w_row[2] = row_of(e.W13_h);
        tp.b2h = e.b12_16; tp.b3h = e.b13_16;
        const size_t row0 = (size_t)(mod_base - p.mod) / CB2_MOD_TOTAL;
        tp.mod16 = p.mod16 + row0 * 768 + layer * 256;
        tp.mod16_stride = mod_stride_b ? 768 : 0;
        tp.res = reinterpret_cast<const __half*>(first ? p.hE0 : p.hE);
        tp.out = reinterpret_cast<__half*>(p.hE);
    } else {
        const DecLayerW& d = m.dec[layer];
        tp.P16 = p.P16[0]; tp.n_w = 2;
        tp.w_row[0] = row_of(d.W1b2_h); tp.w_row[1] = row_of(d.W2_h); tp.b2h = d.b2_16;
    }
    const int grid = min(p.num_sms, tp.n_tiles);
#ifdef CB2_WITH_WG
    static const bool wg_impl = getenv("CB2_EDGE_WG") != nullptr;
    if (wg_impl) {
        const dim3 g(grid), b(wg::WG_CTA_THREADS);
        const size_t sm = wg::wg_smem_bytes(mode);
        if (mode == EDGE_ENC_EDGE) CB2_CUDA(launch_pdl(wg::edge_wg_kernel<EDGE_ENC_EDGE, false>, g, b, sm, s, maps, tp));
        else if (mode == EDGE_ENC_NODE && masked) CB2_CUDA(launch_pdl(wg::edge_wg_kernel<EDGE_ENC_NODE, true>, g, b, sm, s, maps, tp));
        else if (mode == EDGE_ENC_NODE) CB2_CUDA(launch_pdl(wg::edge_wg_kernel<EDGE_ENC_NODE, false>, g, b, sm, s, maps, tp));
        else if (masked) CB2_CUDA(launch_pdl(wg::edge_wg_kernel<EDGE_DEC, true>, g, b, sm, s, maps, tp));
        else CB2_CUDA(launch_pdl(wg::edge_wg_kernel<EDGE_DEC, false>, g, b, sm, s, maps, tp));
        CB2_LAUNCH_CHECK();
        p.launches++;
        return 0;
    }
#endif
    const dim3 g(grid), b(CTA_THREADS);
    const size_t sm = tc_smem_bytes(mode);
    if (mode == EDGE_ENC_EDGE) CB2_CUDA(launch_pdl(edge_tc_kernel<EDGE_ENC_EDGE, false>, g, b, sm, s, maps, tp));
    else if (mode == EDGE_ENC_NODE && masked) CB2_CUDA(launch_pdl(edge_tc_kernel<EDGE_ENC_NODE, true>, g, b, sm, s, maps, tp));
    else if (mode == EDGE_ENC_NODE) CB2_CUDA(launch_pdl(edge_tc_kernel<EDGE_ENC_NODE, false>, g, b, sm, s, maps, tp));
    else if (masked) CB2_CUDA(launch_pdl(edge_tc_kernel<EDGE_DEC, true>, g, b, sm, s, maps, tp));
    else CB2_CUDA(launch_pdl(edge_tc_kernel<EDGE_DEC, false>, g, b, sm, s, maps, tp));
    CB2_LAUNCH_CHECK();
    p.launches++;
    return 0;
}

}
```

codlad_b200/csrc/model.h:

```cpp
#pragma once
#include <cuda_runtime.h>
#include <cuda_fp16.h>
#include <stdint.h>
#include <string>
#include <unordered_map>
#include <vector>

#include "common.cuh"

namespace cb2 {

struct EncLayerW {
    const float *W1a_t, *W1b_t, *W1c_t, *b1, *W2_t, *b2, *W3_t, *b3;
    const float *W11a_t, *W11b_t, *W11c_t, *b11, *W12_t, *b12, *W13_t, *b13;
    const float *Win_t, *bin, *Wout_t, *bout;
    const __half *W1b_h, *W2_h, *W11b_h, *W12_h, *W13_h;
    const __half *W1a_h, *W1c_h, *W11a_h, *W11c_h, *W3_h, *Win_h , *Wout_h ;
    const __half *b2_16, *b12_16, *b13_16;
};

struct DecLayerW {
    const float *W1a_t, *W1b2_t , *W1d_t, *b1, *TS ;
    const float *W2_t, *b2, *W3_t, *b3, *Win_t, *bin, *Wout_t, *bout;
    const __half *W1b2_h, *W2_h;
    const __half *W1a_h, *W1d_h, *W3_h, *Win_h , *Wout_h ;
    const __half* b2_16;
};

struct DenoiserModel {
    int k_neighbors = 64;
    int vocab = 30;
    const float *freqs , *te_w0_t, *te_b0, *te_w2_t, *te_b2, *ada_w_t, *ada_b;
    const float *xin_w_t , *xin_b;
    const float *pos_table, *wedge_t, *ln_w, *ln_b, *we_t, *we_b;
    EncLayerW enc[3];
    DecLayerW dec[3];
    const float *fin_w_t , *fin_b;
    float* dev_f32 = nullptr;
    __half* dev_f16 = nullptr;
    __half* dev_vec16 = nullptr;
    int n_f16_blocks = 0;
};

enum Precision { PREC_F32 = 0, PREC_F16 = 1 };
enum UpdateKind { UPDATE_DDPM = 0, UPDATE_DDIM = 1 };

struct Plan {
    const DenoiserModel* model = nullptr;
    int F = 0, NB = 0, L = 0, K = 0, precision = PREC_F32;
    int T_rows = 0;
    float* X = nullptr;
    int* lengths = nullptr;
    int* cg_z = nullptr;
    int* frame_of = nullptr;
    int* nbr_idx = nullptr;
    float* nbr_dist = nullptr;
    void* hE0 = nullptr;
    float* E_dbg = nullptr;
    void* hE = nullptr;
    float* hV = nullptr;
    float* hVenc = nullptr;
    float* P = nullptr;
    __half* P16[2] = {nullptr, nullptr};
    __half* mod16 = nullptr;
    int num_sms = 148;
    bool all_full = false;
    unsigned long long* tc_trace = nullptr;
    float* silu_c = nullptr;
    float* S = nullptr;
    float* out6 = nullptr;
    float* mod = nullptr;
    int mod_capacity = 0;
    int* mod_row = nullptr;
    float* tvals = nullptr;
    float* coef = nullptr;
    int coef_steps = 0;
    int update_kind = 0;
    bool coef_noisy = true;
    cudaGraphExec_t graph = nullptr;
    const void* graph_key[4] = {nullptr, nullptr, nullptr, nullptr};
    int graph_steps = 0;
    bool graph_all_full = false;
    std::vector<void*> allocs;
    void* tmaps = nullptr;
    void* node_tc = nullptr;
    long long launches = 0;
};

int launch_knn(const float* X, const int* lengths, int F, int L, int K, float* D, int* idx, cudaStream_t s);
int launch_edge_features(const DenoiserModel& m, const float* X, const int* lengths, const int* idx, const float* D,
                         int F, int L, int K, float* E_dbg, void* hE0, int precision, cudaStream_t s);
int launch_edge_raw_features(const float* X, const int* idx, const float* D, int F, int L, int K, float* raw_out, cudaStream_t s);
int launch_timestep_mod(const DenoiserModel& m, const float* tvals, int n, float* scratch_silu_c, float* mod, __half* mod16, cudaStream_t s);
int launch_p_sample(const float* x, const float* out6, const float* noise, const float* coef_rows, const int* step_of_row,
                    int rows_per_b, int n_rows, int C, float* x_next, cudaStream_t s);
int launch_ddim_sample(const float* x, const float* out6, const float* noise, const float* coef_rows, const int* step_of_row,
                       int rows_per_b, int n_rows, int C, float* x_next, cudaStream_t s);
float* plan_P(Plan& p, int which);

struct NodeArgs;
int launch_node_init(Plan& p, const float* x, const float* mod_base, int mod_stride_b, cudaStream_t s);
int launch_node_update(Plan& p, int phase , const float* mod_base, int mod_stride_b,
                       const float* x_t, const float* noise, float* x_next, const float* coef_row, cudaStream_t s);
int launch_edge_f32(Plan& p, int mode, int layer, const float* mod_base, int mod_stride_b, cudaStream_t s);
int launch_edge_tc(Plan& p, int mode, int layer, const float* mod_base, int mod_stride_b, cudaStream_t s);
int edge_tc_prepare(Plan& p);
int node_tc_prepare(Plan& p);
void node_tc_release(Plan& p);
int launch_node_init_tc(Plan& p, const float* x, cudaStream_t s);
int launch_node_update_tc(Plan& p, int phase, const float* mod_base, int mod_stride_b, const float* x_t, const float* noise,
                          float* x_next, const float* coef_row, cudaStream_t s);
void edge_tc_release(Plan& p);
const unsigned int* edge_tc_trap_log();

enum EdgeMode { EDGE_ENC_NODE = 0, EDGE_ENC_EDGE = 1, EDGE_DEC = 2 };

}
```

codlad_b200/csrc/node_tc.cu:

```cuda
#include "node_tc_body.cuh"

namespace cb2 {

using namespace tc;

namespace {

__global__ void __launch_bounds__(NODE_CTA_THREADS, 1) node_tc_kernel(const __grid_constant__ CUtensorMap wmap, const NodeTcParams p) {
    extern __shared__ __align__(1024) unsigned char smem[];
    __shared__ uint32_t s_tmem;
    const int tid = threadIdx.x, warp = tid >> 5;
    if (tid == 0) trace_window(p.trace, p.trace_slot, false);
    if ((smem_u32(smem) & 1023u) != 0) __trap();
    pdl_launch_dependents();
    if (warp == 16) {
        asm volatile("tcgen05.alloc.cta_group::1.sync.aligned.shared::cta.b32 [%0], 512;" ::"r"(smem_u32(&s_tmem)) : "memory");
        asm volatile("tcgen05.relinquish_alloc_permit.cta_group::1.sync.aligned;" ::: "memory");
    }
    tc_fence_before();
    __syncthreads();
    tc_fence_after();
    const uint32_t tmem_base = s_tmem;
    node_block(smem, tmem_base, &wmap, p, blockIdx.x * NT, p.N, true);
    if (tid == 0) trace_window(p.trace, p.trace_slot, true);
    if (warp == 16) asm volatile("tcgen05.dealloc.cta_group::1.sync.aligned.b32 %0, 512;" ::"r"(tmem_base) : "memory");
}


struct NodeTcState { CUtensorMap wmap; };

int node_tc_launch(Plan& p, NodeTcParams& np, cudaStream_t s) {
    const NodeTcState& st = *reinterpret_cast<const NodeTcState*>(p.node_tc);
    CB2_CUDA(launch_pdl(node_tc_kernel, dim3((np.N + NT - 1) / NT), dim3(NODE_CTA_THREADS), NODE_TC_SMEM, s, st.wmap, np));
    CB2_LAUNCH_CHECK();
    p.launches++;
    return 0;
}

void base_params(Plan& p, NodeTcParams& np) {
    np = NodeTcParams{};
    np.N = p.NB * p.L; np.L = p.L; np.K = p.K;
    np.lengths = p.lengths; np.frame_of = p.frame_of; np.nbr_idx = p.nbr_idx; np.cg_z = p.cg_z;
    np.hV = p.hV; np.hVenc = p.hVenc; np.S = p.S;
    np.trace = p.tc_trace; np.trace_slot = p.launches & 2047;
}

}

int node_tc_prepare(Plan& p) {
    EncodeTiledFn fn = nullptr;
    if (get_encode_fn(&fn)) return 1;
    NodeTcState* st = new NodeTcState();
    p.node_tc = st;
    if (encode_rows_map(fn, &st->wmap, p.model->dev_f16, (size_t)p.model->n_f16_blocks * 128, 128)) return 1;
    CB2_CUDA(cudaFuncSetAttribute(node_tc_kernel, cudaFuncAttributeMaxDynamicSharedMemorySize, (int)NODE_TC_SMEM));
    return 0;
}

void node_tc_release(Plan& p) {
    delete reinterpret_cast<NodeTcState*>(p.node_tc);
    p.node_tc = nullptr;
}

int launch_node_init_tc(Plan& p, const float* x, cudaStream_t s) {
    const DenoiserModel& m = *p.model;
    auto row_of = [&](const __half* w) { return (int)((w - m.dev_f16) / 128); };
    NodeTcParams np;
    base_params(p, np);
    np.do_update = 0;
    np.x = x; np.xin_w_t = m.xin_w_t; np.xin_b = m.xin_b;
    np.n_proj = 1;
    np.proj[0] = ProjTc{row_of(m.enc[0].W1a_h), row_of(m.enc[0].W1c_h), m.enc[0].b1, nullptr, p.P16[0], 0};
    return node_tc_launch(p, np, s);
}

void node_tc_update_params(Plan& p, int phase, const float* mod_base, int mod_stride_b, const float* x_t, const float* noise,
                           float* x_next, const float* coef_row, tc::NodeTcParams& np) {
    const DenoiserModel& m = *p.model;
    auto row_of = [&](const __half* w) { return (int)((w - m.dev_f16) / 128); };
    base_params(p, np);
    np.do_update = 1;
    np.mod_stride = mod_stride_b;
    if (phase < 3) {
        const EncLayerW& e = m.enc[phase];
        np.masked_count = 1;
        np.w3_row = row_of(e.W3_h); np.win_row = row_of(e.Win_h); np.wout_row = row_of(e.Wout_h);
        np.b3 = e.b3; np.bin = e.bin; np.bout = e.bout;
        np.mod = mod_base + CB2_MOD_ENC_OFF(phase);
        np.n_proj = 2;
        np.proj[0] = ProjTc{row_of(e.W11a_h), row_of(e.W11c_h), e.b11, nullptr, p.P16[1], 0};
        if (phase < 2) {
            const EncLayerW& nx = m.enc[phase + 1];
            np.proj[1] = ProjTc{row_of(nx.W1a_h), row_of(nx.W1c_h), nx.b1, nullptr, p.P16[0], 0};
        } else {
            const DecLayerW& d = m.dec[0];
            np.write_enc = 1;
            np.proj[1] = ProjTc{row_of(d.W1a_h), row_of(d.W1d_h), d.b1, d.TS, p.P16[0], 2};
        }
    } else {
        const int l = phase - 3;
        const DecLayerW& d = m.dec[l];
        np.masked_count = 0;
        np.w3_row = row_of(d.W3_h); np.win_row = row_of(d.Win_h); np.wout_row = row_of(d.Wout_h);
        np.b3 = d.b3; np.bin = d.bin; np.bout = d.bout;
        np.mod = mod_base + CB2_MOD_DEC_OFF(l);
        if (l < 2) {
            const DecLayerW& nx = m.dec[l + 1];
            np.n_proj = 1;
            np.proj[0] = ProjTc{row_of(nx.W1a_h), row_of(nx.W1d_h), nx.b1, nx.TS, p.P16[0], 1};
        } else {
            np.n_proj = 0;
            np.do_final = 1;
            np.fin_mod = mod_base + CB2_MOD_FIN_OFF;
            np.fin_w_t = m.fin_w_t; np.fin_b = m.fin_b;
            np.out6 = p.out6;
            np.x_t = x_t; np.noise = noise; np.x_next = x_next; np.coef = coef_row;
            np.ddim = p.update_kind == UPDATE_DDIM;
        }
    }
}

int launch_node_update_tc(Plan& p, int phase, const float* mod_base, int mod_stride_b, const float* x_t, const float* noise,
                          float* x_next, const float* coef_row, cudaStream_t s) {
    NodeTcParams np;
    node_tc_update_params(p, phase, mod_base, mod_stride_b, x_t, noise, x_next, coef_row, np);
    return node_tc_launch(p, np, s);
}

}
```

Baseline: 82540.

## Fuse final node update with next step's node init; add optional CTA-pair edge path

The last decoder node update of each sampling step now runs in the same kernel as the next step's node-init projection, which removes one launch per step. The graph launch count is now taken from the capture instead of a fixed 16 per step. The edge tensor-core kernel also gains a compile-time CTA-pair mode (cluster of 2, cta_group::2 MMA with weights split across the pair), but it is off by default. The fused kernel runs node_block twice in sequence within each block, so it relies on each block reading only the x_next rows it wrote itself.

```diff
diff --git a/codlad_b200/csrc/capi.cu b/codlad_b200/csrc/capi.cu
--- a/codlad_b200/csrc/capi.cu
+++ b/codlad_b200/csrc/capi.cu
@@ -487,7 +487,7 @@
 }
 
 int run_forward(Plan& p, const float* x, const float* mod_base, int mod_stride, const float* noise, float* x_next,
-                const float* coef_row, cudaStream_t s, int stop_after = -1) {
+                const float* coef_row, cudaStream_t s, int stop_after = -1, bool init_done = false, bool init_next = false) {
     int n = 0;
     auto done = [&]() { return stop_after >= 0 && ++n >= stop_after; };
     const bool tc = p.precision == PREC_F16 && p.node_tc != nullptr;
@@ -495,8 +495,10 @@
         return tc ? launch_node_update_tc(p, phase, mod_base, mod_stride, xt, nz, xn, cf, s)
                   : launch_node_update(p, phase, mod_base, mod_stride, xt, nz, xn, cf, s);
     };
-    if (int e = tc ? launch_node_init_tc(p, x, s) : launch_node_init(p, x, mod_base, mod_stride, s)) return e;
-    if (done()) return 0;
+    if (!init_done) {
+        if (int e = tc ? launch_node_init_tc(p, x, s) : launch_node_init(p, x, mod_base, mod_stride, s)) return e;
+        if (done()) return 0;
+    }
     for (int l = 0; l < 3; ++l) {
         if (int e = edge_dispatch(p, EDGE_ENC_NODE, l, mod_base, mod_stride, s)) return e;
         if (done()) return 0;
@@ -509,7 +511,11 @@
         if (int e = edge_dispatch(p, EDGE_DEC, l, mod_base, mod_stride, s)) return e;
         if (done()) return 0;
         const bool last = l == 2;
-        if (int e = node_update(3 + l, last ? x : nullptr, last ? noise : nullptr, last ? x_next : nullptr, last ? coef_row : nullptr)) return e;
+        if (last && init_next) {
+            if (int e = launch_node_final_init_tc(p, mod_base, mod_stride, x, noise, x_next, coef_row, s)) return e;
+        } else if (int e = node_update(3 + l, last ? x : nullptr, last ? noise : nullptr, last ? x_next : nullptr, last ? coef_row : nullptr)) {
+            return e;
+        }
         if (done()) return 0;
     }
     return 0;
@@ -573,10 +579,12 @@
     const size_t n3 = (size_t)p.NB * p.L * 3;
     CB2_CUDA(cudaMemcpyAsync(h->xa, x, n3 * sizeof(float), cudaMemcpyDeviceToDevice, s));
     float *cur = h->xa, *nxt = h->xb;
+    const bool fuse_init = p.precision == PREC_F16 && p.node_tc != nullptr;
     for (int step = p.coef_steps - 1; step >= 0; --step) {
         const float* mod_row = p.mod + (size_t)step * CB2_MOD_TOTAL;
         const float* step_noise = noise != nullptr ? noise + (size_t)step * n3 : nullptr;
-        if (int e = run_forward(p, cur, mod_row, 0, step_noise, nxt, p.coef + (size_t)step * 8, s)) {
+        if (int e = run_forward(p, cur, mod_row, 0, step_noise, nxt, p.coef + (size_t)step * 8, s, -1,
+                                fuse_init && step != p.coef_steps - 1, fuse_init && step > 0)) {
             char prev[1024];
             snprintf(prev, sizeof(prev), "%s", g_err);
             const unsigned int* tl = edge_tc_trap_log();
@@ -611,6 +619,7 @@
         int e = enqueue_loop(h, x, noise, cs);
         cudaGraph_t g = nullptr;
         cudaError_t ce = cudaStreamEndCapture(cs, &g);
+        const long long captured = p.launches - before;
         p.launches = before;
         if (e || ce != cudaSuccess) {
             if (g) cudaGraphDestroy(g);
@@ -623,9 +632,10 @@
         cudaStreamDestroy(cs);
         if (ce != cudaSuccess) { set_error("graph instantiate failed: %s", cudaGetErrorString(ce)); p.graph = nullptr; return (int)ce; }
         p.graph_key[0] = x; p.graph_key[1] = noise; p.graph_steps = p.coef_steps; p.graph_all_full = p.all_full;
+        p.graph_launches = captured;
     }
     CB2_CUDA(cudaGraphLaunch(p.graph, s));
-    p.launches += 16LL * p.coef_steps;
+    p.launches += p.graph_launches;
     return 0;
 }
 
diff --git a/codlad_b200/csrc/edge_tc.cu b/codlad_b200/csrc/edge_tc.cu
--- a/codlad_b200/csrc/edge_tc.cu
+++ b/codlad_b200/csrc/edge_tc.cu
@@ -8,7 +8,53 @@
 
 namespace {
 
-constexpr int IND_BYTES = 16 * 128 * 2;
+__device__ __forceinline__ uint32_t cluster_ctarank() {
+    uint32_t r;
+    asm volatile("mov.u32 %0, %%cluster_ctarank;" : "=r"(r));
+    return r;
+}
+__device__ __forceinline__ uint32_t mapa_shared(uint32_t addr, uint32_t rank) {
+    uint32_t d;
+    asm volatile("mapa.shared::cluster.u32 %0, %1, %2;" : "=r"(d) : "r"(addr), "r"(rank));
+    return d;
+}
+__device__ __forceinline__ bool mbar_try_cluster(uint32_t bar, uint32_t parity) {
+    uint32_t done;
+    asm volatile("{\n\t.reg .pred p;\n\tmbarrier.try_wait.parity.acquire.cluster.shared::cta.b64 p, [%1], %2;\n\tselp.u32 %0, 1, 0, p;\n\t}"
+                 : "=r"(done) : "r"(bar), "r"(parity) : "memory");
+    return done != 0;
+}
+static __device__ __noinline__ void mbar_wait_cluster_slow(uint32_t bar, uint32_t parity) {
+    uint32_t spins = 0;
+    while (true) {
+        __nanosleep(64);
+        if (mbar_try_cluster(bar, parity)) return;
+        if (++spins == SPIN_LIMIT) mbar_timeout(bar, parity, false);
+        if (spins > SPIN_LIMIT + (SPIN_LIMIT >> 1)) mbar_timeout(bar, parity, true);
+    }
+}
+__device__ __forceinline__ void mbar_wait_cluster(uint32_t bar, uint32_t parity) {
+    if (!mbar_try_cluster(bar, parity)) mbar_wait_cluster_slow(bar, parity);
+}
+__device__ __forceinline__ void mbar_arrive_cluster(uint32_t cluster_addr) {
+    asm volatile("mbarrier.arrive.release.cluster.shared::cluster.b64 _, [%0];" ::"r"(cluster_addr) : "memory");
+}
+__device__ __forceinline__ void cluster_sync() {
+    asm volatile("barrier.cluster.arrive.release;\n\tbarrier.cluster.wait.acquire;" ::: "memory");
+}
+__device__ __forceinline__ void tma_load_2d_pair(uint32_t dst, const CUtensorMap* map, int c0, int c1, uint32_t cluster_bar) {
+    asm volatile("cp.async.bulk.tensor.2d.cta_group::2.shared::cluster.global.mbarrier::complete_tx::bytes [%0], [%1, {%2, %3}], [%4];"
+                 ::"r"(dst), "l"(map), "r"(c0), "r"(c1), "r"(cluster_bar) : "memory");
+}
+__device__ __forceinline__ void umma_f16_pair(uint32_t tmem_d, uint64_t a, uint64_t b, uint32_t idesc, uint32_t accumulate) {
+    asm volatile("{\n\t.reg .pred p;\n\tsetp.ne.b32 p, %4, 0;\n\ttcgen05.mma.cta_group::2.kind::f16 [%0], %1, %2, %3, p;\n\t}"
+                 ::"r"(tmem_d), "l"(a), "l"(b), "r"(idesc), "r"(accumulate) : "memory");
+}
+__device__ __forceinline__ void umma_commit_pair(uint32_t bar) {
+    asm volatile("tcgen05.commit.cta_group::2.mbarrier::arrive::one.shared::cluster.multicast::cluster.b64 [%0], %1;"
+                 ::"r"(bar), "h"((uint16_t)3) : "memory");
+}
+
 constexpr int MAX_NPT = 4;
 
 struct TcMaps {
@@ -46,6 +92,13 @@
 constexpr int CTA_THREADS = EPI_THREADS + 64;
 constexpr int NSLOT = 4;
 
+#ifndef CB2_EDGE_PAIR
+#define CB2_EDGE_PAIR 0
+#endif
+constexpr bool PAIR = CB2_EDGE_PAIR != 0;
+constexpr int W_BYTES = PAIR ? TILE_BYTES / 2 : TILE_BYTES;
+constexpr int IND_ROWS = PAIR ? 8 : 16;
+
 __device__ __forceinline__ void row_quarter_sync(int q) { asm volatile("bar.sync %0, %1;" ::"r"(q + 1), "n"(32 * NCG) : "memory"); }
 
 struct TileMeta { uint32_t a, b; };
@@ -59,13 +112,15 @@
     extern __shared__ __align__(1024) unsigned char smem[];
     constexpr int N_W = MODE == EDGE_ENC_EDGE ? 3 : 2;
     unsigned char* sW = smem;
-    unsigned char* sT = sW + N_W * TILE_BYTES;
+    unsigned char* sT = sW + N_W * W_BYTES;
     unsigned char* sAux = sT + 4 * TILE_BYTES;
     unsigned char* sInd = sAux;
-    uint64_t* sBar = reinterpret_cast<uint64_t*>(sAux + (MODE == EDGE_ENC_EDGE ? 0 : IND_BYTES));
+    uint64_t* sBar = reinterpret_cast<uint64_t*>(sAux + (MODE == EDGE_ENC_EDGE ? 0 : IND_ROWS * 256));
     uint32_t* sTmem = reinterpret_cast<uint32_t*>(sBar + 29);
 
     const int tid = threadIdx.x;
+    const uint32_t crank = PAIR ? cluster_ctarank() : 0u;
+    auto lead = [&](uint32_t bar) { return PAIR ? mapa_shared(bar, 0) : bar; };
     if (tid == 0) trace_window(p.trace, p.trace_slot, false);
     const int K = p.K, NPT = p.NPT;
     if ((smem_u32(smem) & 1023u) != 0) __trap();
@@ -76,21 +131,26 @@
         for (int g = 0; g < 4; ++g) {
             mbar_init(smem_u32(&sBar[1 + 3 * g]), 1);
             mbar_init(smem_u32(&sBar[2 + 3 * g]), 1);
-            mbar_init(smem_u32(&sBar[3 + 3 * g]), EPI_THREADS / 32);
+            mbar_init(smem_u32(&sBar[3 + 3 * g]), (PAIR && crank == 0 ? 2 : 1) * EPI_THREADS / 32);
             mbar_init(smem_u32(&sBar[13 + g]), 1);
             mbar_init(smem_u32(&sBar[17 + g]), 1);
             mbar_init(smem_u32(&sBar[21 + g]), 1);
-            mbar_init(smem_u32(&sBar[25 + g]), 4);
+            mbar_init(smem_u32(&sBar[25 + g]), PAIR && crank == 0 ? 8 : 4);
         }
         asm volatile("fence.mbarrier_init.release.cluster;" ::: "memory");
     }
     if (tid >= EPI_THREADS && tid < EPI_THREADS + 32) {
-        asm volatile("tcgen05.alloc.cta_group::1.sync.aligned.shared::cta.b32 [%0], 512;" ::"r"(smem_u32(sTmem)) : "memory");
-        asm volatile("tcgen05.relinquish_alloc_permit.cta_group::1.sync.aligned;" ::: "memory");
+        if (PAIR) {
+            asm volatile("tcgen05.alloc.cta_group::2.sync.aligned.shared::cta.b32 [%0], 512;" ::"r"(smem_u32(sTmem)) : "memory");
+            asm volatile("tcgen05.relinquish_alloc_permit.cta_group::2.sync.aligned;" ::: "memory");
+        } else {
+            asm volatile("tcgen05.alloc.cta_group::1.sync.aligned.shared::cta.b32 [%0], 512;" ::"r"(smem_u32(sTmem)) : "memory");
+            asm volatile("tcgen05.relinquish_alloc_permit.cta_group::1.sync.aligned;" ::: "memory");
+        }
     }
     if (MODE != EDGE_ENC_EDGE) {
-        for (int t = tid; t < 16 * 16; t += CTA_THREADS) {
-            const int q = t >> 4, c16 = t & 15;
+        for (int t = tid; t < IND_ROWS * 16; t += CTA_THREADS) {
+            const int ql = t >> 4, c16 = t & 15, q = (int)crank * 8 + ql;
             uint32_t w[4];
 #pragma unroll
             for (int e = 0; e < 4; ++e) {
@@ -99,20 +159,24 @@
                 const __half hi = __float2half((q < NPT && (r0 + 1) / K == q) ? 0.5f : 0.f);
                 w[e] = (uint32_t)__half_as_ushort(lo) | ((uint32_t)__half_as_ushort(hi) << 16);
             }
-            const uint32_t off = (uint32_t)((c16 >> 3) * (16 * 128) + q * 128 + (((c16 & 7) ^ (q & 7)) << 4));
+            const uint32_t off = (uint32_t)((c16 >> 3) * (IND_ROWS * 128) + ql * 128 + (((c16 & 7) ^ (ql & 7)) << 4));
             *reinterpret_cast<uint4*>(sInd + off) = make_uint4(w[0], w[1], w[2], w[3]);
         }
     }
     fence_async_smem();
     tc_fence_before();
-    __syncthreads();
+    if (PAIR) cluster_sync();
+    else __syncthreads();
     tc_fence_after();
     const uint32_t tmem_base = *sTmem;
-    const int tile_begin = (int)((long long)blockIdx.x * p.n_tiles / gridDim.x);
-    const int tile_end = (int)((long long)(blockIdx.x + 1) * p.n_tiles / gridDim.x);
+    const int tile_begin = PAIR ? (int)((long long)(blockIdx.x / 2) * ((p.n_tiles + 1) / 2) / (gridDim.x / 2))
+                                : (int)((long long)blockIdx.x * p.n_tiles / gridDim.x);
+    const int tile_end = PAIR ? (int)((long long)(blockIdx.x / 2 + 1) * ((p.n_tiles + 1) / 2) / (gridDim.x / 2))
+                              : (int)((long long)(blockIdx.x + 1) * p.n_tiles / gridDim.x);
+    auto real_tile = [&](int t) { return PAIR ? 2 * t + (int)crank : t; };
     constexpr int tile_stride = 4;
-    constexpr uint32_t IDESC_MAIN = umma_idesc(128, 128, 0, 0);
-    constexpr uint32_t IDESC_RED = umma_idesc(128, 16, 1, 0);
+    constexpr uint32_t IDESC_MAIN = umma_idesc(PAIR ? 256 : 128, 128, 0, 0);
+    constexpr uint32_t IDESC_RED = umma_idesc(PAIR ? 256 : 128, 16, 1, 0);
 
     if (tid >= EPI_THREADS) {
         auto T_u32 = [&](int g) { return smem_u32(sT + g * TILE_BYTES); };
@@ -139,29 +203,43 @@
         if (tid >= EPI_THREADS + 32) {
             const CUtensorMap* in_map = p.in_is_frame ? &maps.in_frame : &maps.state;
             if (elect_one()) {
-                mbar_expect_tx(smem_u32(&sBar[0]), (uint32_t)(N_W * TILE_BYTES));
+                if (crank == 0) mbar_expect_tx(smem_u32(&sBar[0]), (uint32_t)((PAIR ? 2 : 1) * N_W * W_BYTES));
                 for (int m = 0; m < N_W; ++m)
-                    for (int h = 0; h < 2; ++h)
-                        tma_load_2d(smem_u32(sW + m * TILE_BYTES + h * HALF_BYTES), &maps.weights, h * 64, p.w_row[m], smem_u32(&sBar[0]));
+                    for (int h = 0; h < 2; ++h) {
+                        const uint32_t dst = smem_u32(sW + m * W_BYTES + h * (W_BYTES / 2));
+                        if (PAIR) tma_load_2d_pair(dst, &maps.weights, h * 64, p.w_row[m] + 64 * (int)crank, lead(smem_u32(&sBar[0])));
+                        else tma_load_2d(dst, &maps.weights, h * 64, p.w_row[m], smem_u32(&sBar[0]));
+                    }
             }
             __syncwarp();
             int nv[4], out_row0[4], in_row0[4];
-            auto issue_rows = [&](int g, uint32_t bar) {
+            auto issue_rows = [&](int g, uint32_t bar, bool to_lead, uint32_t lead_bytes) {
                 if (elect_one()) {
-                    mbar_expect_tx(bar, (uint32_t)(nv[g] * K * 256));
+                    if (!(PAIR && to_lead)) mbar_expect_tx(bar, (uint32_t)(nv[g] * K * 256));
+                    else if (crank == 0) mbar_expect_tx(bar, lead_bytes);
+                    const uint32_t cbar = PAIR && to_lead ? lead(bar) : bar;
                     for (int q = 0; q < nv[g]; ++q)
-                        for (int h = 0; h < 2; ++h)
-                            tma_load_2d(T_u32(g) + h * HALF_BYTES + q * K * 128, in_map, h * 64, in_row0[g] + q * K, bar);
+                        for (int h = 0; h < 2; ++h) {
+                            if (PAIR && to_lead) tma_load_2d_pair(T_u32(g) + h * HALF_BYTES + q * K * 128, in_map, h * 64, in_row0[g] + q * K, cbar);
+                            else tma_load_2d(T_u32(g) + h * HALF_BYTES + q * K * 128, in_map, h * 64, in_row0[g] + q * K, bar);
+                        }
                 }
                 __syncwarp();
             };
+            auto nv_of_tile = [&](int tr) {
+                if (tr >= p.n_tiles) return 0;
+                const int b = tr / p.tiles_per_member;
+                return min(NPT, p.L - (tr - b * p.tiles_per_member) * NPT);
+            };
             auto issue_load = [&](int g, int t) {
-                const int b = t / p.tiles_per_member;
-                const int i0 = (t - b * p.tiles_per_member) * NPT;
-                nv[g] = min(NPT, p.L - i0);
+                const int tr = real_tile(t);
+                const bool none = PAIR && tr >= p.n_tiles;
+                const int b = none ? 0 : tr / p.tiles_per_member;
+                const int i0 = none ? 0 : (tr - b * p.tiles_per_member) * NPT;
+                nv[g] = none ? 0 : min(NPT, p.L - i0);
                 in_row0[g] = ((p.in_is_frame ? __ldg(p.frame_of + b) : b) * p.L + i0) * K;
                 out_row0[g] = (b * p.L + i0) * K;
-                issue_rows(g, bar_load(g));
+                issue_rows(g, bar_load(g), true, PAIR ? (uint32_t)((nv[g] + nv_of_tile(tr + 1)) * K * 256) : 0u);
             };
             pdl_wait();
             for (int g = 0; g < 4; ++g)
@@ -169,12 +247,13 @@
             uint32_t ph_go = 0;
             for (int t0 = tile_begin; t0 < tile_end; t0 += tile_stride) {
                 if (MODE == EDGE_ENC_EDGE) {
-                    for (int g = 0; g < 4 && t0 + g < tile_end; ++g) { mbar_wait(bar_m3(g), ph_go); issue_rows(g, bar_res(g)); }
+                    for (int g = 0; g < 4 && t0 + g < tile_end; ++g) { mbar_wait(bar_m3(g), ph_go); issue_rows(g, bar_res(g), false, 0u); }
                 }
                 for (int g = 0; g < 4; ++g) {
                     const int t = t0 + g;
                     if (t >= tile_end) break;
-                    mbar_wait(bar_go(g), ph_go);
+                    if (PAIR) mbar_wait_cluster(bar_go(g), ph_go);
+                    else mbar_wait(bar_go(g), ph_go);
                     cmark(0, g);
                     if (MODE == EDGE_ENC_EDGE) {
                         if (elect_one()) {
@@ -194,18 +273,31 @@
                 ph_go ^= 1;
             }
             if (MODE == EDGE_ENC_EDGE) { if (elect_one()) tma_store_wait_all(); __syncwarp(); }
-        } else {
+        } else if (crank == 0) {
             uint32_t ph_epi = 0;
+            auto mma = [&](uint32_t d, uint64_t a, uint64_t b, uint32_t idesc, uint32_t acc) {
+                if (PAIR) umma_f16_pair(d, a, b, idesc, acc);
+                else umma_f16(d, a, b, idesc, acc);
+            };
+            auto commit = [&](uint32_t bar) {
+                if (PAIR) umma_commit_pair(bar);
+                else umma_commit(bar);
+            };
+            auto wait = [&](uint32_t bar, uint32_t parity) {
+                if (PAIR) mbar_wait_cluster(bar, parity);
+                else mbar_wait(bar, parity);
+            };
             auto issue_mma = [&](int g, int w_slot) {
                 tc_fence_after();
-                const uint64_t a0 = umma_desc(T_u32(g), 16, 1024), b0 = umma_desc(smem_u32(sW + w_slot * TILE_BYTES), 16, 1024);
+                const uint64_t a0 = umma_desc(T_u32(g), 16, 1024), b0 = umma_desc(smem_u32(sW + w_slot * W_BYTES), 16, 1024);
                 if (elect_one()) {
 #pragma unroll
                     for (int k = 0; k < 8; ++k) {
                         const uint64_t koff = (uint64_t)(((k >> 2) * HALF_BYTES + (k & 3) * 32) >> 4);
-                        umma_f16(tmem_base + (uint32_t)(g * 128), a0 + koff, b0 + koff, IDESC_MAIN, k > 0);
-                    }
-                    umma_commit(bar_acc(g));
+                        const uint64_t kofb = (uint64_t)(((k >> 2) * (W_BYTES / 2) + (k & 3) * 32) >> 4);
+                        mma(tmem_base + (uint32_t)(g * 128), a0 + koff, b0 + kofb, IDESC_MAIN, k > 0);
+                    }
+                    commit(bar_acc(g));
                 }
                 __syncwarp();
             };
@@ -215,15 +307,15 @@
                 if (elect_one()) {
 #pragma unroll
                     for (int k = 0; k < 8; ++k)
-                        umma_f16(tmem_base + (uint32_t)(g * 128), a0 + (uint64_t)((k * 16 * 128) >> 4),
-                                 b0 + (uint64_t)(((k >> 2) * (16 * 128) + (k & 3) * 32) >> 4), IDESC_RED, k > 0);
-                    umma_commit(bar_acc(g));
-                    umma_commit(bar_go(g));
+                        mma(tmem_base + (uint32_t)(g * 128), a0 + (uint64_t)((k * 16 * 128) >> 4),
+                            b0 + (uint64_t)(((k >> 2) * (IND_ROWS * 128) + (k & 3) * 32) >> 4), IDESC_RED, k > 0);
+                    commit(bar_acc(g));
+                    commit(bar_go(g));
                 }
                 __syncwarp();
             };
             cmark(6, 0);
-            mbar_wait(smem_u32(&sBar[0]), 0);
+            wait(smem_u32(&sBar[0]), 0);
             cmark(7, 0);
             uint32_t round = 0;
             if (MODE == EDGE_ENC_EDGE) {
@@ -231,35 +323,38 @@
                     const int n = min(4, tile_end - t0);
                     const int n_next = max(0, min(4, tile_end - (t0 + tile_stride)));
                     if (round == 0)
-                        for (int g = 0; g < n; ++g) { mbar_wait(bar_load(g), 0); issue_mma(g, 0); }
-                    for (int g = 0; g < n; ++g) { mbar_wait(bar_epi(g), ph_epi); cmark(0, g); issue_mma(g, 1); cmark(1, g); }
+                        for (int g = 0; g < n; ++g) { wait(bar_load(g), 0); issue_mma(g, 0); }
+                    for (int g = 0; g < n; ++g) { wait(bar_epi(g), ph_epi); cmark(0, g); issue_mma(g, 1); cmark(1, g); }
                     ph_epi ^= 1;
                     for (int g = 0; g < n; ++g) {
-                        mbar_wait(bar_epi(g), ph_epi);
+                        wait(bar_epi(g), ph_epi);
                         cmark(2, g);
                         issue_mma(g, 2);
-                        if (elect_one()) umma_commit(bar_m3(g));
+                        if (elect_one()) commit(bar_m3(g));
                         __syncwarp();
                     }
                     ph_epi ^= 1;
                     const uint32_t next_parity = (round + 1) & 1;
                     for (int g = 0; g < n; ++g) {
-                        mbar_wait(bar_epi(g), ph_epi);
-                        if (elect_one()) mbar_arrive(bar_go(g));
+                        wait(bar_epi(g), ph_epi);
+                        if (elect_one()) {
+                            mbar_arrive(bar_go(g));
+                            if (PAIR) mbar_arrive_cluster(mapa_shared(bar_go(g), 1));
+                        }
                         __syncwarp();
                         cmark(3, g);
-                        if (g >= 1 && g - 1 < n_next) { mbar_wait(bar_load(g - 1), next_parity); cmark(4, g - 1); issue_mma(g - 1, 0); cmark(5, g - 1); }
-                    }
-                    if (n - 1 < n_next) { mbar_wait(bar_load(n - 1), next_parity); issue_mma(n - 1, 0); }
+                        if (g >= 1 && g - 1 < n_next) { wait(bar_load(g - 1), next_parity); cmark(4, g - 1); issue_mma(g - 1, 0); cmark(5, g - 1); }
+                    }
+                    if (n - 1 < n_next) { wait(bar_load(n - 1), next_parity); issue_mma(n - 1, 0); }
                     ph_epi ^= 1;
                 }
             } else {
                 bool pend3 = false;
                 uint32_t pend_round = 0;
                 auto restart = [&](int h, uint32_t rnd) {
-                    mbar_wait(smem_u32(&sBar[25 + h]), rnd & 1);
+                    wait(smem_u32(&sBar[25 + h]), rnd & 1);
                     cmark(3, h);
-                    mbar_wait(bar_load(h), (rnd + 1) & 1);
+                    wait(bar_load(h), (rnd + 1) & 1);
                     cmark(4, h);
                     issue_mma(h, 0);
                     cmark(5, h);
@@ -268,14 +363,14 @@
                     const int n = min(4, tile_end - t0);
                     const int n_next = max(0, min(4, tile_end - (t0 + tile_stride)));
                     if (round == 0)
-                        for (int g = 0; g < n; ++g) { mbar_wait(bar_load(g), 0); issue_mma(g, 0); }
+                        for (int g = 0; g < n; ++g) { wait(bar_load(g), 0); issue_mma(g, 0); }
                     for (int g = 0; g < n; ++g) {
-                        mbar_wait(bar_epi(g), ph_epi); cmark(0, g); issue_mma(g, 1); cmark(1, g);
+                        wait(bar_epi(g), ph_epi); cmark(0, g); issue_mma(g, 1); cmark(1, g);
                         if (g == 0 && pend3) { restart(3, pend_round); pend3 = false; }
                     }
                     ph_epi ^= 1;
                     for (int g = 0; g < n; ++g) {
-                        mbar_wait(bar_epi(g), ph_epi);
+                        wait(bar_epi(g), ph_epi);
                         cmark(2, g);
                         issue_reduce(g);
                         if (g >= 1 && g - 1 < n_next) restart(g - 1, round);
@@ -298,13 +393,17 @@
             if (wrote_smem) fence_async_smem();
             tc_fence_before();
             __syncwarp();
-            if ((tid & 31) == 0) mbar_arrive(smem_u32(&sBar[3 + 3 * s]));
-        };
-
-        const int step_b = tile_stride / p.tiles_per_member, step_t = tile_stride - step_b * p.tiles_per_member;
+            if ((tid & 31) == 0) {
+                if (PAIR) mbar_arrive_cluster(lead(smem_u32(&sBar[3 + 3 * s])));
+                else mbar_arrive(smem_u32(&sBar[3 + 3 * s]));
+            }
+        };
+
+        constexpr int real_stride = PAIR ? 2 * tile_stride : tile_stride;
+        const int step_b = real_stride / p.tiles_per_member, step_t = real_stride - step_b * p.tiles_per_member;
         auto make_meta = [&](int tile, int b, int tin) {
             TileMeta m{((uint32_t)b << 16) | (uint32_t)tin, 0x80000000u};
-            if (tile >= tile_end) { m.a = 0u; return m; }
+            if (tile >= tile_end || (PAIR && real_tile(tile) >= p.n_tiles)) { m.a = 0u; return m; }
             const int i0 = tin * NPT;
             const int f = p.single_frame ? 0 : __ldg(p.frame_of + b);
             if (q_of_r < min(NPT, p.L - i0))
@@ -312,8 +411,8 @@
             return m;
         };
         auto first_meta = [&](int tile) {
-            const int b = tile / p.tiles_per_member;
-            return make_meta(tile, b, tile - b * p.tiles_per_member);
+            const int b = real_tile(tile) / p.tiles_per_member;
+            return make_meta(tile, b, real_tile(tile) - b * p.tiles_per_member);
         };
         auto next_meta = [&](const TileMeta& m, int tile) {
             int b = meta_member(m) + step_b, tin = meta_tin(m) + step_t;
@@ -365,6 +464,7 @@
         auto drain = [&](int s, int next_tile) {
             const TileMeta m = m3;
             m3 = next_meta(m, next_tile);
+            const bool tile_ok = !PAIR || real_tile(next_tile - tile_stride) < p.n_tiles;
             if (cq == s % NCG) {
                 mark(8, s);
                 mbar_wait(smem_u32(&sBar[2 + 3 * s]), ph ^ 1);
@@ -375,10 +475,13 @@
                 const int nv = nv_of(m), node0 = node0_of(m);
 #pragma unroll
                 for (int q = 0; q < MAX_NPT; ++q)
-                    if (q < nv) p.S[((size_t)node0 + q) * 128 + r] = s4[q];
+                    if (q < nv && tile_ok) p.S[((size_t)node0 + q) * 128 + r] = s4[q];
                 tc_fence_before();
                 __syncwarp();
-                if ((tid & 31) == 0) mbar_arrive(smem_u32(&sBar[25 + s]));
+                if ((tid & 31) == 0) {
+                    mbar_arrive(smem_u32(&sBar[25 + s]));
+                    if (PAIR && crank != 0) mbar_arrive_cluster(lead(smem_u32(&sBar[25 + s])));
+                }
                 mark(10, s);
             }
         };
@@ -588,12 +691,16 @@
             ph ^= 1;
             ph_res ^= 1;
         }
-        if (MODE != EDGE_ENC_EDGE && pending3) drain(3, tile_end);
+        if (MODE != EDGE_ENC_EDGE && pending3) drain(3, tile_end + 3);
     }
     tc_fence_before();
-    __syncthreads();
+    if (PAIR) cluster_sync();
+    else __syncthreads();
     if (tid == 0) trace_window(p.trace, p.trace_slot, true);
-    if (tid >= EPI_THREADS && tid < EPI_THREADS + 32) asm volatile("tcgen05.dealloc.cta_group::1.sync.aligned.b32 %0, 512;" ::"r"(tmem_base) : "memory");
+    if (tid >= EPI_THREADS && tid < EPI_THREADS + 32) {
+        if (PAIR) asm volatile("tcgen05.dealloc.cta_group::2.sync.aligned.b32 %0, 512;" ::"r"(tmem_base) : "memory");
+        else asm volatile("tcgen05.dealloc.cta_group::1.sync.aligned.b32 %0, 512;" ::"r"(tmem_base) : "memory");
+    }
 }
 
 }
@@ -606,8 +713,25 @@
 
 size_t tc_smem_bytes(int mode) {
     const int n_w = mode == EDGE_ENC_EDGE ? 3 : 2;
-    return (size_t)(n_w + 4) * TILE_BYTES + (mode == EDGE_ENC_EDGE ? 0 : IND_BYTES) + 29 * 8 + 16;
-}
+    return (size_t)n_w * W_BYTES + 4 * TILE_BYTES + (mode == EDGE_ENC_EDGE ? 0 : IND_ROWS * 256) + 29 * 8 + 16;
+}
+
+template <typename... KArgs, typename... Args>
+inline cudaError_t launch_pdl_cluster(void (*kernel)(KArgs...), dim3 grid, dim3 block, size_t smem, cudaStream_t stream, int cluster, Args&&... args) {
+    if (cluster == 1) return launch_pdl(kernel, grid, block, smem, stream, std::forward<Args>(args)...);
+    cudaLaunchConfig_t cfg{};
+    cfg.gridDim = grid; cfg.blockDim = block; cfg.dynamicSmemBytes = smem; cfg.stream = stream;
+    static const bool no_pdl = getenv("CB2_NO_PDL") != nullptr;
+    cudaLaunchAttribute attr[2];
+    attr[0].id = cudaLaunchAttributeProgrammaticStreamSerialization;
+    attr[0].val.programmaticStreamSerializationAllowed = no_pdl ? 0 : 1;
+    attr[1].id = cudaLaunchAttributeClusterDimension;
+    attr[1].val.clusterDim.x = (unsigned)cluster; attr[1].val.clusterDim.y = 1; attr[1].val.clusterDim.z = 1;
+    cfg.attrs = attr; cfg.numAttrs = 2;
+    return cudaLaunchKernelEx(&cfg, kernel, std::forward<Args>(args)...);
+}
+
+int g_max_pairs = 0;
 
 }
 
@@ -623,7 +747,7 @@
     p.tmaps = m;
     if (encode_rows_map(fn, &m->in_frame, p.hE0, (size_t)p.F * p.L * p.K, p.K)) return 1;
     if (encode_rows_map(fn, &m->state, p.hE, (size_t)p.NB * p.L * p.K, p.K)) return 1;
-    if (encode_rows_map(fn, &m->weights, p.model->dev_f16, (size_t)p.model->n_f16_blocks * 128, 128)) return 1;
+    if (encode_rows_map(fn, &m->weights, p.model->dev_f16, (size_t)p.model->n_f16_blocks * 128, PAIR ? 64 : 128)) return 1;
     if (getenv("CB2_TRAP_DEBUG") != nullptr && g_trap_host == nullptr) {
         unsigned int* dptr = nullptr;
         CB2_CUDA(cudaHostAlloc(&g_trap_host, 256, cudaHostAllocMapped));
@@ -639,6 +763,16 @@
     CB2_CUDA(cudaFuncSetAttribute(edge_tc_kernel<EDGE_DEC, false>, cudaFuncAttributeMaxDynamicSharedMemorySize, (int)tc_smem_bytes(EDGE_DEC)));
     CB2_CUDA(cudaFuncSetAttribute(edge_tc_kernel<EDGE_DEC, true>, cudaFuncAttributeMaxDynamicSharedMemorySize, (int)tc_smem_bytes(EDGE_DEC)));
     CB2_CUDA(cudaFuncSetAttribute(edge_tc_kernel<EDGE_ENC_EDGE, false>, cudaFuncAttributeMaxDynamicSharedMemorySize, (int)tc_smem_bytes(EDGE_ENC_EDGE)));
+    if (PAIR && g_max_pairs == 0) {
+        cudaLaunchConfig_t cfg{};
+        cfg.gridDim = dim3(2); cfg.blockDim = dim3(CTA_THREADS); cfg.dynamicSmemBytes = tc_smem_bytes(EDGE_ENC_EDGE);
+        cudaLaunchAttribute attr[1];
+        attr[0].id = cudaLaunchAttributeClusterDimension;
+        attr[0].val.clusterDim.x = 2; attr[0].val.clusterDim.y = 1; attr[0].val.clusterDim.z = 1;
+        cfg.attrs = attr; cfg.numAttrs = 1;
+        CB2_CUDA(cudaOccupancyMaxActiveClusters(&g_max_pairs, edge_tc_kernel<EDGE_ENC_EDGE, false>, &cfg));
+        if (g_max_pairs < 1) { set_error("edge_tc: no CTA pair fits"); return 1; }
+    }
 #ifdef CB2_WITH_WG
     CB2_CUDA(cudaFuncSetAttribute(wg::edge_wg_kernel<EDGE_ENC_NODE, false>, cudaFuncAttributeMaxDynamicSharedMemorySize, (int)wg::wg_smem_bytes(EDGE_ENC_NODE)));
     CB2_CUDA(cudaFuncSetAttribute(wg::edge_wg_kernel<EDGE_ENC_NODE, true>, cudaFuncAttributeMaxDynamicSharedMemorySize, (int)wg::wg_smem_bytes(EDGE_ENC_NODE)));
@@ -707,13 +841,14 @@
         return 0;
     }
 #endif
-    const dim3 g(grid), b(CTA_THREADS);
+    const dim3 g(PAIR ? 2 * min(g_max_pairs, (tp.n_tiles + 1) / 2) : grid), b(CTA_THREADS);
     const size_t sm = tc_smem_bytes(mode);
-    if (mode == EDGE_ENC_EDGE) CB2_CUDA(launch_pdl(edge_tc_kernel<EDGE_ENC_EDGE, false>, g, b, sm, s, maps, tp));
-    else if (mode == EDGE_ENC_NODE && masked) CB2_CUDA(launch_pdl(edge_tc_kernel<EDGE_ENC_NODE, true>, g, b, sm, s, maps, tp));
-    else if (mode == EDGE_ENC_NODE) CB2_CUDA(launch_pdl(edge_tc_kernel<EDGE_ENC_NODE, false>, g, b, sm, s, maps, tp));
-    else if (masked) CB2_CUDA(launch_pdl(edge_tc_kernel<EDGE_DEC, true>, g, b, sm, s, maps, tp));
-    else CB2_CUDA(launch_pdl(edge_tc_kernel<EDGE_DEC, false>, g, b, sm, s, maps, tp));
+    const int cl = PAIR ? 2 : 1;
+    if (mode == EDGE_ENC_EDGE) CB2_CUDA(launch_pdl_cluster(edge_tc_kernel<EDGE_ENC_EDGE, false>, g, b, sm, s, cl, maps, tp));
+    else if (mode == EDGE_ENC_NODE && masked) CB2_CUDA(launch_pdl_cluster(edge_tc_kernel<EDGE_ENC_NODE, true>, g, b, sm, s, cl, maps, tp));
+    else if (mode == EDGE_ENC_NODE) CB2_CUDA(launch_pdl_cluster(edge_tc_kernel<EDGE_ENC_NODE, false>, g, b, sm, s, cl, maps, tp));
+    else if (masked) CB2_CUDA(launch_pdl_cluster(edge_tc_kernel<EDGE_DEC, true>, g, b, sm, s, cl, maps, tp));
+    else CB2_CUDA(launch_pdl_cluster(edge_tc_kernel<EDGE_DEC, false>, g, b, sm, s, cl, maps, tp));
     CB2_LAUNCH_CHECK();
     p.launches++;
     return 0;
diff --git a/codlad_b200/csrc/model.h b/codlad_b200/csrc/model.h
--- a/codlad_b200/csrc/model.h
+++ b/codlad_b200/csrc/model.h
@@ -80,6 +80,7 @@
     cudaGraphExec_t graph = nullptr;
     const void* graph_key[4] = {nullptr, nullptr, nullptr, nullptr};
     int graph_steps = 0;
+    long long graph_launches = 0;
     bool graph_all_full = false;
     std::vector<void*> allocs;
     void* tmaps = nullptr;
@@ -108,6 +109,8 @@
 int node_tc_prepare(Plan& p);
 void node_tc_release(Plan& p);
 int launch_node_init_tc(Plan& p, const float* x, cudaStream_t s);
+int launch_node_final_init_tc(Plan& p, const float* mod_base, int mod_stride_b, const float* x_t, const float* noise, float* x_next,
+                              const float* coef_row, cudaStream_t s);
 int launch_node_update_tc(Plan& p, int phase, const float* mod_base, int mod_stride_b, const float* x_t, const float* noise,
                           float* x_next, const float* coef_row, cudaStream_t s);
 void edge_tc_release(Plan& p);
diff --git a/codlad_b200/csrc/node_tc.cu b/codlad_b200/csrc/node_tc.cu
--- a/codlad_b200/csrc/node_tc.cu
+++ b/codlad_b200/csrc/node_tc.cu
@@ -26,6 +26,27 @@
     if (warp == 16) asm volatile("tcgen05.dealloc.cta_group::1.sync.aligned.b32 %0, 512;" ::"r"(tmem_base) : "memory");
 }
 
+__global__ void __launch_bounds__(NODE_CTA_THREADS, 1) node_tc_final_init_kernel(const __grid_constant__ CUtensorMap wmap, const NodeTcParams p,
+                                                                                 const NodeTcParams q) {
+    extern __shared__ __align__(1024) unsigned char smem[];
+    __shared__ uint32_t s_tmem;
+    const int tid = threadIdx.x, warp = tid >> 5;
+    if (tid == 0) trace_window(p.trace, p.trace_slot, false);
+    if ((smem_u32(smem) & 1023u) != 0) __trap();
+    pdl_launch_dependents();
+    if (warp == 16) {
+        asm volatile("tcgen05.alloc.cta_group::1.sync.aligned.shared::cta.b32 [%0], 512;" ::"r"(smem_u32(&s_tmem)) : "memory");
+        asm volatile("tcgen05.relinquish_alloc_permit.cta_group::1.sync.aligned;" ::: "memory");
+    }
+    tc_fence_before();
+    __syncthreads();
+    tc_fence_after();
+    const uint32_t tmem_base = s_tmem;
+    node_block(smem, tmem_base, &wmap, p, blockIdx.x * NT, p.N, true);
+    node_block(smem, tmem_base, &wmap, q, blockIdx.x * NT, q.N, false);
+    if (tid == 0) trace_window(p.trace, p.trace_slot, true);
+    if (warp == 16) asm volatile("tcgen05.dealloc.cta_group::1.sync.aligned.b32 %0, 512;" ::"r"(tmem_base) : "memory");
+}
 
 struct NodeTcState { CUtensorMap wmap; };
 
@@ -54,6 +75,7 @@
     p.node_tc = st;
     if (encode_rows_map(fn, &st->wmap, p.model->dev_f16, (size_t)p.model->n_f16_blocks * 128, 128)) return 1;
     CB2_CUDA(cudaFuncSetAttribute(node_tc_kernel, cudaFuncAttributeMaxDynamicSharedMemorySize, (int)NODE_TC_SMEM));
+    CB2_CUDA(cudaFuncSetAttribute(node_tc_final_init_kernel, cudaFuncAttributeMaxDynamicSharedMemorySize, (int)NODE_TC_SMEM));
     return 0;
 }
 
@@ -62,15 +84,19 @@
     p.node_tc = nullptr;
 }
 
-int launch_node_init_tc(Plan& p, const float* x, cudaStream_t s) {
+static void node_tc_init_params(Plan& p, const float* x, NodeTcParams& np) {
     const DenoiserModel& m = *p.model;
     auto row_of = [&](const __half* w) { return (int)((w - m.dev_f16) / 128); };
-    NodeTcParams np;
     base_params(p, np);
     np.do_update = 0;
     np.x = x; np.xin_w_t = m.xin_w_t; np.xin_b = m.xin_b;
     np.n_proj = 1;
     np.proj[0] = ProjTc{row_of(m.enc[0].W1a_h), row_of(m.enc[0].W1c_h), m.enc[0].b1, nullptr, p.P16[0], 0};
+}
+
+int launch_node_init_tc(Plan& p, const float* x, cudaStream_t s) {
+    NodeTcParams np;
+    node_tc_init_params(p, x, np);
     return node_tc_launch(p, np, s);
 }
 
@@ -120,6 +146,18 @@
     }
 }
 
+int launch_node_final_init_tc(Plan& p, const float* mod_base, int mod_stride_b, const float* x_t, const float* noise, float* x_next,
+                              const float* coef_row, cudaStream_t s) {
+    NodeTcParams np, ni;
+    node_tc_update_params(p, 5, mod_base, mod_stride_b, x_t, noise, x_next, coef_row, np);
+    node_tc_init_params(p, x_next, ni);
+    const NodeTcState& st = *reinterpret_cast<const NodeTcState*>(p.node_tc);
+    CB2_CUDA(launch_pdl(node_tc_final_init_kernel, dim3((np.N + NT - 1) / NT), dim3(NODE_CTA_THREADS), NODE_TC_SMEM, s, st.wmap, np, ni));
+    CB2_LAUNCH_CHECK();
+    p.launches++;
+    return 0;
+}
+
 int launch_node_update_tc(Plan& p, int phase, const float* mod_base, int mod_stride_b, const float* x_t, const float* noise,
                           float* x_next, const float* coef_row, cudaStream_t s) {
     NodeTcParams np;
```

Measured after the change: 82060 (median of 6 runs). Within noise of the previous version (-0.6%).
